# refresh-bio/KMC

Measured on NVIDIA H100. Metric: stage-2 k-mers/s (k=31), higher is better.
Workload: dtype u64

## Files before the change

kmc_b200/csrc/expand.cuh:

```cuda
#pragma once
#include "common.cuh"

#ifndef KMCB200_EXPAND_UNROLL
#define KMCB200_EXPAND_UNROLL 8
#endif

namespace kmcb {

constexpr int kExpandUnroll = KMCB200_EXPAND_UNROLL;

#ifndef KMCB200_EXPAND_IPT
#define KMCB200_EXPAND_IPT 8
#endif
template <int WORDS> struct ExpandCfg { static constexpr int kTile = WORDS == 1 ? 4096 : 2048, kThreads = WORDS == 1 ? 4096 / KMCB200_EXPAND_IPT : 256; };
constexpr int kExpandMinTile = 2048;

struct ExpandArgs {
	const uint8_t* bin;
	uint64_t size;
	const uint64_t* pack_start;
	uint32_t n_packs;
	uint32_t k;
	uint32_t min_rec_bytes;
	uint32_t tile;
	uint32_t both_strands;
	uint64_t n_rec;
	uint32_t* sk_off;
	uint32_t* sk_kpre;
	uint32_t* tile_first;
	uint32_t* pack_nsk;
	uint32_t* pack_nk;
	uint64_t* pack_kbase;
	uint32_t* pack_tbase;
	uint32_t* tile_pack;
	uint4* tile_desc;
	uint64_t tile_pack_cap;
	uint32_t* status;
	uint32_t* flags;
	void* recs;
	uint16_t* cells1;
	uint64_t* item_lo1;
	uint16_t* item_cnt1;
	uint32_t top_shift;
	const uint32_t* cell_scan;
	uint32_t mode;
	uint32_t fshift, fprefix, fmask;
	uint64_t* hist12;
	unsigned long long* out_counter;
	const uint16_t* blk_of_prefix;
	const uint64_t* region_start;
	uint32_t n_blocks;
};
enum : uint32_t { kExpandAll = 0, kExpandCount12 = 1, kExpandFilter = 2, kExpandScatter = 3, kExpandCells = 4, kExpandPartition = 5 };
template <int WORDS> __host__ __device__ constexpr bool expand_partition_supported() { return WORDS == 1; }
constexpr uint32_t kExpandMaxBlocks = 512;
constexpr uint64_t kExpandUnknownRecs = ~0ull;

enum : uint32_t { kErrPackWalk = 1, kErrRecCount = 2 };
constexpr uint32_t kExpandAbortFlag = 2;

__device__ __forceinline__ uint64_t tile_first_base(uint64_t pack_start, uint32_t p, uint32_t tile) { return pack_start * 4 / tile + p; }

constexpr int kWalkSegBytes = 256;
constexpr int kWalkSegs = 256;
constexpr int kWalkChunk = kWalkSegBytes * kWalkSegs;
#ifndef KMCB200_WALK_SPEC
#define KMCB200_WALK_SPEC 1024
#endif
constexpr int kWalkSpec = KMCB200_WALK_SPEC;

__global__ void __launch_bounds__(kWalkSegs, 3) walk_packs_parallel_kernel(const ExpandArgs a, uint32_t* pack_done)
{
	extern __shared__ __align__(16) uint8_t wsm[];
	__shared__ uint32_t s_entry[kWalkSegs], s_exit[kWalkSegs], s_w[16];
	__shared__ uint32_t s_bad;
	const uint32_t p = blockIdx.x, tid = threadIdx.x, lane = tid & 31, warp = tid >> 5;
	const uint64_t pstart = a.pack_start[p];
	const uint32_t len = (uint32_t)min(a.pack_start[p + 1] - pstart, (uint64_t)kWalkChunk + 1);
	if (len > (uint32_t)kWalkChunk || len == 0) { if (tid == 0) pack_done[p] = len == 0 ? 1u : 0u; if (len == 0 && tid == 0) { a.pack_nsk[p] = 0; a.pack_nk[p] = 0; } return; }
	{
		const uintptr_t g0 = reinterpret_cast<uintptr_t>(a.bin + pstart);
		const uintptr_t g0a = g0 & ~(uintptr_t)15;
		const uint32_t shift = (uint32_t)(g0 - g0a);
		const uint32_t nvec = (len + shift + 15) >> 4;
		for (uint32_t v0 = tid; v0 < nvec; v0 += 8 * kWalkSegs) {
			uint4 r[8];
#pragma unroll
			for (int i = 0; i < 8; ++i) { const uint32_t v = v0 + i * kWalkSegs; r[i] = v < nvec ? __ldg(reinterpret_cast<const uint4*>(g0a) + v) : make_uint4(0, 0, 0, 0); }
#pragma unroll
			for (int i = 0; i < 8; ++i) { const uint32_t v = v0 + i * kWalkSegs; if (v < nvec) reinterpret_cast<uint4*>(wsm)[v] = r[i]; }
		}
		if (tid == 0) s_bad = 0;
		__syncthreads();
		const uint8_t* pk = wsm + shift;
		const uint32_t k3 = a.k + 3;
		const uint32_t seg_lo = tid * kWalkSegBytes, seg_hi = min(seg_lo + (uint32_t)kWalkSegBytes, len);
		uint32_t pos = seg_lo > (uint32_t)kWalkSpec ? seg_lo - kWalkSpec : 0;
		if (seg_lo < len) {
			while (pos < seg_lo) pos += 1 + ((pk[pos] + k3) >> 2);
		} else pos = len;
		uint32_t entry = min(pos, len);
		uint32_t nrec = 0, nk = 0;
		pos = entry;
		while (pos < seg_hi) { const uint32_t x = pk[pos]; nk += x + 1; ++nrec; pos += 1 + ((x + k3) >> 2); }
		s_entry[tid] = entry; s_exit[tid] = seg_lo < len ? pos : len;
		for (int it = 0; it < kWalkSegs; ++it) {
			__syncthreads();
			const uint32_t want = tid > 0 ? min(s_exit[tid - 1], len) : 0u;
			const bool fix = tid > 0 && seg_lo < len && entry != want;
			if (!__syncthreads_or(fix)) break;
			if (fix) {
				entry = want; nrec = 0; nk = 0; pos = entry;
				while (pos < seg_hi) { const uint32_t x = pk[pos]; nk += x + 1; ++nrec; pos += 1 + ((x + k3) >> 2); }
				s_entry[tid] = entry; s_exit[tid] = pos;
			}
		}
		__syncthreads();
		bool bad = false;
		if (tid > 0 && seg_lo < len && s_entry[tid] != min(s_exit[tid - 1], len)) bad = true;
		if (tid == kWalkSegs - 1 || seg_hi == len) { if (seg_lo < len && s_exit[tid] != len) bad = true; }
		if (bad) atomicOr(&s_bad, 1u);
		uint32_t ir = nrec, ik = nk;
#pragma unroll
		for (int o = 1; o < 32; o <<= 1) {
			const uint32_t tr = __shfl_up_sync(0xffffffffu, ir, o), tk = __shfl_up_sync(0xffffffffu, ik, o);
			if (lane >= (uint32_t)o) { ir += tr; ik += tk; }
		}
		if (lane == 31) { s_w[warp] = ir; s_w[8 + warp] = ik; }
		__syncthreads();
		if (s_bad) {
			if (tid == 0) { atomicOr(a.status, kErrPackWalk); a.pack_nsk[p] = 0; a.pack_nk[p] = 0; pack_done[p] = 1; }
			return;
		}
		uint32_t br = ir - nrec, bk = ik - nk, tr = 0, tk = 0;
#pragma unroll
		for (int w = 0; w < 8; ++w) { if ((uint32_t)w < warp) { br += s_w[w]; bk += s_w[8 + w]; } tr += s_w[w]; tk += s_w[8 + w]; }
		const uint64_t slot = pstart / a.min_rec_bytes;
		const uint64_t tfb = tile_first_base(pstart, p, a.tile);
		uint32_t j = br, kk = bk;
		pos = entry;
		while (pos < seg_hi) {
			const uint32_t x = pk[pos];
			a.sk_off[slot + j] = (uint32_t)(pstart + pos);
			a.sk_kpre[slot + j] = kk;
			const uint32_t tb = (kk + a.tile - 1) / a.tile;
			if (tb * a.tile < kk + x + 1) a.tile_first[tfb + tb] = j;
			kk += x + 1;
			pos += 1 + ((x + k3) >> 2);
			++j;
		}
		if (tid == 0) { a.pack_nsk[p] = tr; a.pack_nk[p] = tk; pack_done[p] = 1; }
	}
}

constexpr int kWalkWarpsPerBlock = 4;

__device__ __forceinline__ uint4 walk_load_window(const uint8_t* bin_aligned, uint64_t wbase, uint64_t limit, uint32_t lane)
{
	const uint64_t o = wbase + 16ull * lane;
	return o < limit ? __ldg(reinterpret_cast<const uint4*>(bin_aligned + o)) : make_uint4(0, 0, 0, 0);
}

__global__ void __launch_bounds__(32 * kWalkWarpsPerBlock) walk_packs_kernel(const ExpandArgs a, const uint32_t* pack_done)
{
	const uint32_t lane = threadIdx.x & 31u;
	const uint32_t p = blockIdx.x * kWalkWarpsPerBlock + (threadIdx.x >> 5);
	if (p >= a.n_packs) return;
	if (pack_done && pack_done[p]) return;
	uint64_t pos = a.pack_start[p];
	const uint64_t end = a.pack_start[p + 1];
	const uint64_t slot = pos / a.min_rec_bytes;
	const uint64_t tfb = tile_first_base(pos, p, a.tile);
	const uintptr_t base_addr = reinterpret_cast<uintptr_t>(a.bin);
	const uint8_t* bin_aligned = reinterpret_cast<const uint8_t*>(base_addr & ~(uintptr_t)15);
	const uint64_t shift = base_addr & 15u;
	const uint64_t limit = ((a.size + shift + 15) & ~15ull);
	uint64_t wbase = (pos + shift) & ~511ull;
	uint4 cur = walk_load_window(bin_aligned, wbase, limit, lane);
	uint4 nxt = walk_load_window(bin_aligned, wbase + 512, limit, lane);
	uint32_t j = 0, nk = 0, next_tile = 0;
	uint32_t my_off = 0, my_kpre = 0;
	while (pos < end) {
		uint64_t rel = pos + shift - wbase;
		if (rel >= 512) {
			cur = nxt;
			wbase += 512;
			nxt = walk_load_window(bin_aligned, wbase + 512, limit, lane);
			rel -= 512;
		}
		const uint32_t r = (uint32_t)rel;
		const uint32_t comp = (r >> 2) & 3u;
		uint32_t w = comp == 0 ? cur.x : comp == 1 ? cur.y : comp == 2 ? cur.z : cur.w;
		w = __shfl_sync(0xffffffffu, w, r >> 4);
		const uint32_t x = (w >> ((r & 3u) * 8u)) & 0xFFu;
		if (lane == (j & 31u)) { my_off = (uint32_t)pos; my_kpre = nk; }
		if ((j & 31u) == 31u) {
			a.sk_off[slot + j - 31 + lane] = my_off;
			a.sk_kpre[slot + j - 31 + lane] = my_kpre;
		}
		if (nk + x + 1 > next_tile * a.tile) {
			if (lane == 0) a.tile_first[tfb + next_tile] = j;
			++next_tile;
		}
		nk += x + 1;
		pos += 1 + ((x + a.k + 3) >> 2);
		++j;
	}
	if (lane < (j & 31u)) {
		a.sk_off[slot + (j & ~31u) + lane] = my_off;
		a.sk_kpre[slot + (j & ~31u) + lane] = my_kpre;
	}
	if (lane == 0) {
		if (pos != end) atomicOr(a.status, kErrPackWalk);
		a.pack_nsk[p] = j;
		a.pack_nk[p] = nk;
	}
}

__global__ void __launch_bounds__(1024) index_from_extras_kernel(const ExpandArgs a, const uint8_t* __restrict__ extras, const uint64_t* __restrict__ pack_rec_start)
{
	__shared__ uint32_t s_b[32], s_k[32];
	__shared__ uint32_t carry_b, carry_k;
	__shared__ uint32_t s_bad;
	const uint32_t p = blockIdx.x, tid = threadIdx.x, lane = tid & 31, warp = tid >> 5;
	const uint64_t pstart = a.pack_start[p];
	const uint32_t len = (uint32_t)min(a.pack_start[p + 1] - pstart, (uint64_t)0xffffffffu);
	const uint64_t r0 = pack_rec_start[p];
	const uint32_t nrec = (uint32_t)min(pack_rec_start[p + 1] - r0, (uint64_t)0xffffffffu);
	const uint64_t slot = pstart / a.min_rec_bytes;
	const uint64_t tfb = tile_first_base(pstart, p, a.tile);
	if (tid == 0) { carry_b = 0; carry_k = 0; s_bad = 0; }
	__syncthreads();
	const bool too_many = (uint64_t)nrec * a.min_rec_bytes > (uint64_t)len;
	for (uint32_t j0 = 0; j0 < nrec && !too_many; j0 += 1024) {
		const uint32_t j = j0 + tid;
		const uint32_t x = j < nrec ? extras[r0 + j] : 0u;
		const uint32_t nb = j < nrec ? 1u + ((x + a.k + 3u) >> 2) : 0u, nk = j < nrec ? x + 1u : 0u;
		uint32_t ib = nb, ik = nk;
#pragma unroll
		for (int o = 1; o < 32; o <<= 1) {
			const uint32_t tb = __shfl_up_sync(0xffffffffu, ib, o), tk = __shfl_up_sync(0xffffffffu, ik, o);
			if (lane >= (uint32_t)o) { ib += tb; ik += tk; }
		}
		if (lane == 31) { s_b[warp] = ib; s_k[warp] = ik; }
		__syncthreads();
		uint32_t bb = carry_b, bk = carry_k;
		for (uint32_t w = 0; w < warp; ++w) { bb += s_b[w]; bk += s_k[w]; }
		const uint32_t off = bb + ib - nb, kk = bk + ik - nk;
		if (j < nrec) {
			if (off + nb > len || a.bin[pstart + off] != (uint8_t)x) atomicOr(&s_bad, 1u);
			else {
				a.sk_off[slot + j] = (uint32_t)(pstart + off);
				a.sk_kpre[slot + j] = kk;
				const uint32_t tb = (kk + a.tile - 1) / a.tile;
				if (tb * a.tile < kk + x + 1) a.tile_first[tfb + tb] = j;
			}
		}
		__syncthreads();
		if (tid == 1023) { carry_b = bb + ib; carry_k = bk + ik; }
		__syncthreads();
	}
	if (tid == 0) {
		const bool bad = too_many || s_bad || carry_b != len;
		if (bad) atomicOr(a.status, kErrPackWalk);
		a.pack_nsk[p] = bad ? 0u : nrec;
		a.pack_nk[p] = bad ? 0u : carry_k;
	}
}

__global__ void __launch_bounds__(1024) scan_packs_kernel(const ExpandArgs a)
{
	__shared__ uint64_t s_k[32];
	__shared__ uint32_t s_t[32];
	__shared__ uint64_t carry_k;
	__shared__ uint32_t carry_t;
	const uint32_t tid = threadIdx.x, lane = tid & 31, warp = tid >> 5;
	if (tid == 0) { carry_k = 0; carry_t = 0; }
	__syncthreads();
	const bool walk_failed = (a.status[0] & kErrPackWalk) != 0;
	for (uint32_t base = 0; base < a.n_packs && !walk_failed; base += 1024) {
		const uint32_t p = base + tid;
		const uint32_t nk = p < a.n_packs ? a.pack_nk[p] : 0;
		const uint32_t nt = (nk + a.tile - 1) / a.tile;
		uint64_t ik = nk;
		uint32_t it = nt;
#pragma unroll
		for (int o = 1; o < 32; o <<= 1) {
			uint64_t tk = __shfl_up_sync(0xffffffffu, ik, o);
			uint32_t tt = __shfl_up_sync(0xffffffffu, it, o);
			if (lane >= (uint32_t)o) { ik += tk; it += tt; }
		}
		if (lane == 31) { s_k[warp] = ik; s_t[warp] = it; }
		__syncthreads();
		uint64_t bk = carry_k;
		uint32_t bt = carry_t;
		for (uint32_t w = 0; w < warp; ++w) { bk += s_k[w]; bt += s_t[w]; }
		const uint64_t ek = bk + ik - nk;
		const uint32_t et = bt + it - nt;
		if (p < a.n_packs) {
			a.pack_kbase[p] = ek;
			a.pack_tbase[p] = et;
			for (uint32_t t = 0; t < nt && (uint64_t)et + t < a.tile_pack_cap; ++t) a.tile_pack[et + t] = p;
		}
		__syncthreads();
		if (tid == 1023) { carry_k = ek + nk; carry_t = et + nt; }
		__syncthreads();
	}
	if (tid == 0) {
		a.pack_kbase[a.n_packs] = carry_k;
		a.pack_tbase[a.n_packs] = carry_t;
		bool bad = walk_failed;
		if (a.n_rec != kExpandUnknownRecs && carry_k != a.n_rec) { atomicOr(a.status, kErrRecCount); bad = true; }
		if ((uint64_t)carry_t > a.tile_pack_cap) bad = true;
		a.status[1] = bad ? 0u : carry_t;
		if (bad && a.flags) { atomicOr(&a.flags[0], kExpandAbortFlag); atomicOr(&a.flags[1], kExpandAbortFlag); }
	}
}

__global__ void __launch_bounds__(256) tile_desc_kernel(const ExpandArgs a)
{
	const uint32_t g = blockIdx.x * 256 + threadIdx.x;
	if (g >= a.status[1]) return;
	const uint32_t p = a.tile_pack[g];
	const uint32_t t = g - a.pack_tbase[p];
	const uint64_t pstart = a.pack_start[p];
	const uint64_t slot0 = pstart / a.min_rec_bytes;
	const uint32_t nk = a.pack_nk[p];
	const uint32_t tile_start = t * a.tile;
	const uint32_t cnt = min(a.tile, nk - tile_start);
	const uint32_t j_lo = a.tile_first[tile_first_base(pstart, p, a.tile) + t];
	const uint64_t obase = a.pack_kbase[p] + tile_start;
	a.tile_desc[2 * (size_t)g] = make_uint4((uint32_t)slot0, a.pack_nsk[p], j_lo, a.sk_off[slot0 + j_lo]);
	a.tile_desc[2 * (size_t)g + 1] = make_uint4(tile_start | (cnt - 1u), (uint32_t)a.pack_start[p + 1], (uint32_t)obase, (uint32_t)(obase >> 32));
}

__device__ __forceinline__ uint64_t bswap64(uint64_t x)
{
	const uint32_t lo = (uint32_t)x, hi = (uint32_t)(x >> 32);
	return ((uint64_t)__byte_perm(lo, 0, 0x0123) << 32) | (uint64_t)__byte_perm(hi, 0, 0x0123);
}
__device__ __forceinline__ uint64_t rev_symbols64(uint64_t x)
{
	const uint64_t y = __brevll(x);
	return ((y >> 1) & 0x5555555555555555ull) | ((y & 0x5555555555555555ull) << 1);
}

template <int WORDS, typename Load8>
__device__ __forceinline__ Rec<WORDS> extract_kmer(const uint8_t* payload, uint32_t s, uint32_t k, bool canonical, Load8 load8)
{
	const uint8_t* A = payload + (s >> 2);
	const uint32_t sh = (s & 3u) * 2u;
	const uintptr_t a0 = reinterpret_cast<uintptr_t>(A) & ~(uintptr_t)7;
	const uint32_t bo = (uint32_t)(reinterpret_cast<uintptr_t>(A) - a0) * 8u + sh;
	const uintptr_t need_end = reinterpret_cast<uintptr_t>(A) + ((sh + 2u * k + 7u) >> 3);
	uint64_t b[WORDS + 1];
#pragma unroll
	for (int i = 0; i <= WORDS; ++i) {
		const uintptr_t wa = a0 + 8u * i;
		b[i] = wa < need_end ? bswap64(load8(wa)) : 0ull;
	}
	uint64_t t[WORDS];
#pragma unroll
	for (int i = 0; i < WORDS; ++i) t[i] = bo ? ((b[i] << bo) | (b[i + 1] >> (64u - bo))) : b[i];
	const uint32_t rs = 64u * WORDS - 2u * k;
	Rec<WORDS> f;
#pragma unroll
	for (int i = 0; i < WORDS; ++i) {
		uint64_t v = t[i] >> rs;
		if (i > 0 && rs) v |= t[i - 1] << (64u - rs);
		f.w[WORDS - 1 - i] = v;
	}
	if (!canonical) return f;
	uint64_t u[WORDS];
#pragma unroll
	for (int i = 0; i < WORDS; ++i) u[i] = ~rev_symbols64(f.w[i]);
	Rec<WORDS> r;
#pragma unroll
	for (int i = 0; i < WORDS; ++i) {
		uint64_t v = u[i] >> rs;
		if (i > 0 && rs) v |= u[i - 1] << (64u - rs);
		r.w[WORDS - 1 - i] = v;
	}
	return rec_less<WORDS>(f, r) ? f : r;
}

template <int WORDS>
__device__ __forceinline__ Rec<WORDS> extract_kmer_be32(const uint32_t* sw, uint32_t B, uint32_t k, bool canonical)
{
	const uint32_t wi = B >> 5, bo = B & 31u;
	uint32_t w[2 * WORDS + 1];
#pragma unroll
	for (int i = 0; i <= 2 * WORDS; ++i) w[i] = sw[wi + i];
	uint64_t t[WORDS];
#pragma unroll
	for (int i = 0; i < WORDS; ++i)
		t[i] = ((uint64_t)__funnelshift_l(w[2 * i + 1], w[2 * i], bo) << 32) | (uint64_t)__funnelshift_l(w[2 * i + 2], w[2 * i + 1], bo);
	const uint32_t rs = 64u * WORDS - 2u * k;
	Rec<WORDS> f;
#pragma unroll
	for (int i = 0; i < WORDS; ++i) {
		uint64_t v = t[i] >> rs;
		if (i > 0 && rs) v |= t[i - 1] << (64u - rs);
		f.w[WORDS - 1 - i] = v;
	}
	if (!canonical) return f;
	uint64_t u[WORDS];
#pragma unroll
	for (int i = 0; i < WORDS; ++i) u[i] = ~rev_symbols64(f.w[i]);
	Rec<WORDS> r;
#pragma unroll
	for (int i = 0; i < WORDS; ++i) {
		uint64_t v = u[i] >> rs;
		if (i > 0 && rs) v |= u[i - 1] << (64u - rs);
		r.w[WORDS - 1 - i] = v;
	}
	return rec_less<WORDS>(f, r) ? f : r;
}

template <int WORDS>
__device__ __forceinline__ uint32_t rec_top_digit(const Rec<WORDS>& r, uint32_t shift)
{
	const uint32_t wi = shift >> 6, off = shift & 63u;
	uint64_t lo = r.w[0], hi = 0;
#pragma unroll
	for (int i = 1; i < WORDS; ++i) {
		if (wi == (uint32_t)i) lo = r.w[i];
		if (wi + 1 == (uint32_t)i) hi = r.w[i];
	}
	uint64_t v = lo >> off;
	if (WORDS > 1 && off) v |= hi << (64u - off);
	return (uint32_t)v & 0xFFu;
}

template <int WORDS>
__device__ __forceinline__ uint32_t msd_free_bits(const Rec<WORDS>& r, uint32_t shift, uint32_t mask)
{
	if (WORDS == 1) return (uint32_t)(r.w[0] >> shift) & mask;
	const uint32_t wi = shift >> 6, off = shift & 63u;
	uint64_t lo = r.w[0], hi = 0;
#pragma unroll
	for (int i = 1; i < WORDS; ++i) {
		if (wi == (uint32_t)i) lo = r.w[i];
		if (wi + 1 == (uint32_t)i) hi = r.w[i];
	}
	uint64_t v = lo >> off;
	if (off) v |= hi << (64u - off);
	return (uint32_t)v & mask;
}

template <int WORDS, uint32_t MODE>
__host__ __device__ constexpr int expand_min_blocks() { return MODE == kExpandPartition ? 3 : WORDS <= 2 ? 2048 / ExpandCfg<WORDS>::kThreads : 6; }

template <int WORDS, uint32_t MODE = kExpandAll>
__global__ void __launch_bounds__(ExpandCfg<WORDS>::kThreads, expand_min_blocks<WORDS, MODE>()) expand_kernel(const ExpandArgs a)
{
	constexpr int kExpandTile = ExpandCfg<WORDS>::kTile, kExpandThreads = ExpandCfg<WORDS>::kThreads;
	constexpr int IPT = kExpandTile / kExpandThreads;
	constexpr int MAXSK = 1024, STAGE = 12288;
	constexpr int HW = kExpandTile / 32;
	constexpr int SBYTES = MODE == kExpandPartition && kExpandTile * 8 * WORDS > STAGE + 32 ? kExpandTile * 8 * WORDS : STAGE + 32;
	static_assert(MODE != kExpandPartition || expand_partition_supported<WORDS>(), "kExpandPartition: one-word records only");
	__shared__ uint32_t hbits[HW];
	__shared__ uint32_t hpre[HW];
	__shared__ uint32_t s_bit[MAXSK];
	__shared__ __align__(16) uint8_t s_bytes[SBYTES];
	__shared__ uint32_t s_jmax;
	__shared__ unsigned long long s_fbase;
	__shared__ uint32_t warp_max[kExpandThreads / 32];
	__shared__ uint32_t htop[256];
	static_assert(HW <= 128 && HW % 32 == 0, "the head bitmap is scanned by one warp, HW / 32 words per lane");
	const uint32_t tid = threadIdx.x, lane = tid & 31, warp = tid >> 5;
	const uint32_t le_mask = 0xffffffffu >> (31u - lane);
	static_assert(kExpandThreads % 32 == 0, "output slot i * threads + tid belongs to lane tid % 32");
	if constexpr (MODE == kExpandPartition)
		if (a.flags[1] & kExpandAbortFlag) return;
	if (tid < 256) htop[tid] = 0;
	const uint32_t total_tiles = a.status[1];
	Rec<WORDS>* __restrict__ out = reinterpret_cast<Rec<WORDS>*>(a.recs);

	for (uint32_t g = blockIdx.x; g < total_tiles; g += gridDim.x) {
		uint32_t digit_base = 0;
		if constexpr (MODE == kExpandPartition)
			if (tid < 256) digit_base = __ldg(a.cell_scan + g + (size_t)tid * total_tiles);
		const uint4 da = __ldg(a.tile_desc + 2 * (size_t)g), db = __ldg(a.tile_desc + 2 * (size_t)g + 1);
		if (g + gridDim.x < total_tiles) asm volatile("prefetch.global.L2 [%0];" ::"l"(a.tile_desc + 2 * (size_t)(g + gridDim.x)));
		const uint64_t slot0 = da.x;
		const uint32_t nsk = da.y;
		const uint32_t j_lo = da.z;
		const uint32_t off_lo = da.w;
		const uint32_t tile_start = db.x & ~(uint32_t)(kExpandTile - 1);
		const uint32_t cnt = (db.x & (uint32_t)(kExpandTile - 1)) + 1u;
		const uint32_t* __restrict__ kpre = a.sk_kpre + slot0;
		const uint32_t* __restrict__ off = a.sk_off + slot0;
		const uintptr_t g0a = reinterpret_cast<uintptr_t>(a.bin + off_lo) & ~(uintptr_t)15;
		const uint32_t base_off = (uint32_t)(reinterpret_cast<uintptr_t>(a.bin + off_lo) - g0a);

		__syncthreads();
		if (tid < (uint32_t)HW) hbits[tid] = 0;
		if (tid == 0) s_jmax = j_lo;
		__syncthreads();
		{
			uint32_t jm = j_lo;
			for (uint32_t j = j_lo + tid; j < nsk; j += kExpandThreads) {
				const uint32_t kp = kpre[j];
				if (j > j_lo && kp >= tile_start + cnt) break;
				const uint32_t rel = j - j_lo;
				if (rel < (uint32_t)MAXSK) s_bit[rel] = 8u * (base_off + (off[j] - off_lo) + 1u) + 2u * tile_start - 2u * kp;
				if (j > j_lo) atomicOr(&hbits[(kp - tile_start) >> 5], 1u << ((kp - tile_start) & 31u));
				jm = j;
			}
			if (jm > j_lo) atomicMax(&s_jmax, jm);
		}
		__syncthreads();
		const uint32_t j_hi = s_jmax;
		const uint64_t b_hi = j_hi + 1 < nsk ? (uint64_t)off[j_hi + 1] : (uint64_t)db.y;
		const uint64_t span = reinterpret_cast<uintptr_t>(a.bin + b_hi) - g0a;
		const bool staged = (j_hi - j_lo) < (uint32_t)MAXSK && span + 16 <= (uint64_t)STAGE;
		if (staged)
			for (uint32_t v = tid; v * 16 < span + 8; v += kExpandThreads) {
				uint4 x = __ldg(reinterpret_cast<const uint4*>(g0a) + v);
				x.x = __byte_perm(x.x, 0, 0x0123); x.y = __byte_perm(x.y, 0, 0x0123); x.z = __byte_perm(x.z, 0, 0x0123); x.w = __byte_perm(x.w, 0, 0x0123);
				reinterpret_cast<uint4*>(s_bytes)[v] = x;
			}
		if (warp == 0) {
			constexpr int WPL = HW / 32;
			uint32_t c[WPL], tot = 0;
#pragma unroll
			for (int i = 0; i < WPL; ++i) { c[i] = __popc(hbits[lane * WPL + i]); tot += c[i]; }
			uint32_t inc = tot;
#pragma unroll
			for (int o = 1; o < 32; o <<= 1) {
				const uint32_t x = __shfl_up_sync(0xffffffffu, inc, o);
				if (lane >= (uint32_t)o) inc += x;
			}
			uint32_t ex = inc - tot;
#pragma unroll
			for (int i = 0; i < WPL; ++i) { hpre[lane * WPL + i] = ex; ex += c[i]; }
		}
		__syncthreads();

		const uint64_t obase = ((uint64_t)db.w << 32) | db.z;
		auto kmer_of = [&](uint32_t slot) -> Rec<WORDS> {
			const uint32_t rel = hpre[slot >> 5] + __popc(hbits[slot >> 5] & le_mask);
			if (staged) return extract_kmer_be32<WORDS>(reinterpret_cast<const uint32_t*>(s_bytes), s_bit[rel] + 2u * slot, a.k, a.both_strands != 0);
			const uint32_t j = j_lo + rel;
			const uint32_t s = tile_start + slot - kpre[j];
			return extract_kmer<WORDS>(a.bin + off[j] + 1, s, a.k, a.both_strands != 0,
				[](uintptr_t wa) { return __ldg(reinterpret_cast<const unsigned long long*>(wa)); });
		};
		auto top_digit_of = [&](uint32_t slot) -> uint32_t {
			if (WORDS > 1 || !staged || a.top_shift + 8u != 2u * a.k) return rec_top_digit<WORDS>(kmer_of(slot), a.top_shift);
			const uint32_t rel = hpre[slot >> 5] + __popc(hbits[slot >> 5] & le_mask);
			const uint32_t B = s_bit[rel] + 2u * slot;
			const uint32_t* sw = reinterpret_cast<const uint32_t*>(s_bytes);
			auto byte_at = [&](uint32_t b) { const uint32_t wi = b >> 5; return __funnelshift_l(sw[wi + 1], sw[wi], b & 31u) >> 24; };
			const uint32_t f = byte_at(B);
			if (!a.both_strands) return f;
			uint32_t r = ~byte_at(B + 2u * a.k - 8u) & 0xFFu;
			r = ((r & 0x03u) << 6) | ((r & 0x0Cu) << 2) | ((r & 0x30u) >> 2) | ((r & 0xC0u) >> 6);
			return min(f, r);
		};
		if constexpr (MODE == kExpandAll || MODE == kExpandCells) {
#pragma unroll kExpandUnroll
			for (int i = 0; i < IPT; ++i) {
				const uint32_t slot = i * kExpandThreads + tid;
				if (slot < cnt) {
					if constexpr (MODE == kExpandAll) {
						const Rec<WORDS> r = kmer_of(slot);
						out[obase + slot] = r;
						atomicAdd(&htop[rec_top_digit<WORDS>(r, a.top_shift)], 1u);
					} else atomicAdd(&htop[top_digit_of(slot)], 1u);
				}
			}
			__syncthreads();
			if (tid < 256) {
				a.cells1[(uint64_t)tid * total_tiles + g] = (uint16_t)htop[tid];
				htop[tid] = 0;
			}
			if (tid == 0) { a.item_lo1[g] = obase; a.item_cnt1[g] = (uint16_t)cnt; }
		} else if constexpr (MODE == kExpandPartition) {
			__shared__ uint32_t s_excl[256], s_goff[256];
			Rec<WORDS> key[IPT];
			uint32_t rank[IPT / 2] = {};
#pragma unroll
			for (int i = 0; i < IPT; ++i) {
				const uint32_t slot = i * kExpandThreads + tid;
				if (slot < cnt) {
					key[i] = kmer_of(slot);
					rank[i / 2] |= atomicAdd(&htop[rec_top_digit<WORDS>(key[i], a.top_shift)], 1u) << (16 * (i & 1));
				}
			}
			__syncthreads();
			uint32_t c = 0, inc = 0;
			if (tid < 256) {
				c = htop[tid];
				htop[tid] = 0;
				inc = c;
#pragma unroll
				for (int o = 1; o < 32; o <<= 1) {
					const uint32_t x = __shfl_up_sync(0xffffffffu, inc, o);
					if (lane >= (uint32_t)o) inc += x;
				}
				if (lane == 31) warp_max[warp] = inc;
			}
			__syncthreads();
			if (tid < 256) {
				uint32_t ex = inc - c;
#pragma unroll
				for (int w = 0; w < 8; ++w) if ((uint32_t)w < warp) ex += warp_max[w];
				s_excl[tid] = ex;
				s_goff[tid] = digit_base - ex;
			}
			__syncthreads();
			Rec<WORDS>* buf = reinterpret_cast<Rec<WORDS>*>(s_bytes);
#pragma unroll
			for (int i = 0; i < IPT; ++i) {
				const uint32_t slot = i * kExpandThreads + tid;
				if (slot < cnt) buf[s_excl[rec_top_digit<WORDS>(key[i], a.top_shift)] + ((rank[i / 2] >> (16 * (i & 1))) & 0xFFFFu)] = key[i];
			}
			__syncthreads();
#pragma unroll
			for (int i = 0; i < IPT; ++i) {
				const uint32_t q = i * kExpandThreads + tid;
				if (q < cnt) {
					const Rec<WORDS> r = buf[q];
					out[s_goff[rec_top_digit<WORDS>(r, a.top_shift)] + q] = r;
				}
			}
		} else if constexpr (MODE == kExpandCount12) {
			for (int i = 0; i < IPT; ++i) {
				const uint32_t slot = i * kExpandThreads + tid;
				if (slot < cnt) {
					const Rec<WORDS> r = kmer_of(slot);
					atomicAdd(reinterpret_cast<unsigned long long*>(a.hist12) + msd_free_bits<WORDS>(r, a.fshift, 0xFFFu), 1ull);
				}
			}
		} else if constexpr (MODE == kExpandScatter) {
			__shared__ uint32_t s_bcnt[kExpandMaxBlocks];
			__shared__ unsigned long long s_bbase[kExpandMaxBlocks];
			for (uint32_t b = tid; b < a.n_blocks; b += kExpandThreads) s_bcnt[b] = 0;
			__syncthreads();
			uint16_t blk[IPT], rnk[IPT];
#pragma unroll
			for (int i = 0; i < IPT; ++i) {
				const uint32_t slot = i * kExpandThreads + tid;
				if (slot < cnt) {
					const Rec<WORDS> r = kmer_of(slot);
					blk[i] = a.blk_of_prefix[msd_free_bits<WORDS>(r, a.fshift, 0xFFFu)];
					if (blk[i] != 0xFFFFu) rnk[i] = (uint16_t)atomicAdd(&s_bcnt[blk[i]], 1u);
				}
			}
			__syncthreads();
			for (uint32_t b = tid; b < a.n_blocks; b += kExpandThreads) {
				const uint32_t c = s_bcnt[b];
				if (c) s_bbase[b] = a.region_start[b] + atomicAdd(a.out_counter + b, (unsigned long long)c);
			}
			__syncthreads();
#pragma unroll
			for (int i = 0; i < IPT; ++i) {
				const uint32_t slot = i * kExpandThreads + tid;
				if (slot < cnt && blk[i] != 0xFFFFu) out[s_bbase[blk[i]] + rnk[i]] = kmer_of(slot);
			}
		} else {
			for (int i = 0; i < IPT; ++i) {
				const uint32_t slot = i * kExpandThreads + tid;
				Rec<WORDS> r;
				bool keep = false;
				if (slot < cnt) { r = kmer_of(slot); keep = msd_free_bits<WORDS>(r, a.fshift, a.fmask) == a.fprefix; }
				const uint32_t bal = __ballot_sync(0xffffffffu, keep);
				__syncthreads();
				if (lane == 0) warp_max[warp] = __popc(bal);
				__syncthreads();
				if (tid == 0) {
					uint32_t tot = 0;
					for (int w = 0; w < kExpandThreads / 32; ++w) { const uint32_t c = warp_max[w]; warp_max[w] = tot; tot += c; }
					s_fbase = tot ? atomicAdd(a.out_counter, (unsigned long long)tot) : 0ull;
				}
				__syncthreads();
				if (keep) out[s_fbase + warp_max[warp] + __popc(bal & lanemask_lt())] = r;
			}
		}
	}
}

}
```

kmc_b200/csrc/kmc_b200.cu:

```cuda
#include "../../include/kmc_b200.h"
#include "common.cuh"
#include "expand.cuh"
#include "radix_sort.cuh"
#include "count.cuh"
#include "msd_sort.cuh"
#include "leaf_warp.cuh"
#include "leaf_hash.cuh"
#include "leaf_hash_cta.cuh"
#include "leaf_hash_wide.cuh"
#include "split.cuh"
#include "fastx.cuh"
#include "small_k.cuh"

#include <cmath>
#include <cstddef>
#include <cstdarg>
#include <cstdio>
#include <cstdlib>
#include <cstring>
#include <string>
#include <vector>
#include <algorithm>
#include <list>
#include <thread>

using namespace kmcb;

namespace {

constexpr int kMaxPasses = 4 * 8;
constexpr int kHistRows = kMaxPasses + 1;
constexpr int kCounterSlots = kMaxPasses + 8;
constexpr uint32_t kEpochLimit = (1u << 22) - 2;
constexpr int kStageRing = 4;
constexpr size_t kMaxLeaves = 256 * 1024;
constexpr uint32_t kHeavyListCap = 2048;

thread_local std::string g_create_error;

enum { kHistNone = 0, kHistTiles = 1, kHistCells = 2 };

struct ZeroBlock {
	uint64_t hist[kHistRows][256];
	uint32_t counters[kCounterSlots];
	uint32_t status[2];
	uint32_t msd_flags[4];
	uint32_t msd_n_items[2];
	uint32_t msd_counters[4];
	uint32_t heavy_count[2];
	uint32_t heavy_list[kHeavyListCap];
	uint32_t leaf_group_sum[kMaxLeaves / 1024];
};

static_assert(sizeof(ZeroBlock) % 4 == 0, "zeroed word by word");

struct Slot {
	cudaStream_t stream = nullptr;
	uint8_t* recs_a = nullptr; size_t recs_a_cap = 0;
	uint8_t* recs_b = nullptr; size_t recs_b_cap = 0;
	uint8_t* recs_x = nullptr; size_t recs_x_cap = 0;
	uint8_t* d_bin = nullptr; size_t bin_cap = 0;
	uint64_t* d_pack_start = nullptr; size_t packs_cap = 0;
	uint64_t* h_pack_start[kStageRing] = {}; cudaEvent_t ev_pack[kStageRing] = {}; int ring = 0;
	uint32_t* pack_nsk = nullptr; uint32_t* pack_nk = nullptr; uint32_t* pack_tbase = nullptr; uint64_t* pack_kbase = nullptr;
	uint32_t* pack_done = nullptr;
	uint32_t* sk_off = nullptr; size_t sk_off_cap = 0;
	uint32_t* sk_kpre = nullptr; size_t sk_kpre_cap = 0;
	uint32_t* tile_first = nullptr; size_t tile_first_cap = 0;
	uint32_t* tile_pack = nullptr; size_t tile_pack_cap = 0;
	uint4* tile_desc = nullptr; size_t tile_desc_cap = 0;
	ZeroBlock* zero = nullptr;
	uint64_t* desc = nullptr; size_t desc_cap = 0;
	uint64_t* msd_seg1 = nullptr;
	uint64_t* msd_start2 = nullptr;
	uint64_t* msd_start3 = nullptr;
	uint32_t* msd_item_base1 = nullptr;
	uint32_t* msd_item_base2 = nullptr;
	uint32_t* msd_item_seg2 = nullptr; size_t msd_item_seg2_cap = 0;
	uint64_t* msd_item_lo1 = nullptr; size_t msd_item_lo1_cap = 0;
	uint16_t* msd_item_cnt1 = nullptr; size_t msd_item_cnt1_cap = 0;
	uint16_t* msd_cells = nullptr; size_t msd_cells_cap = 0;
	uint32_t* msd_cell_scan = nullptr; size_t msd_cell_scan_cap = 0;
	uint32_t* msd_block_sums = nullptr; size_t msd_block_sums_cap = 0;
	uint8_t* leaf_tmp = nullptr; size_t leaf_tmp_cap = 0;
	uint32_t* leaf_emit = nullptr; uint64_t* leaf_off = nullptr;
	const char* pass_names[kMaxPasses + 8] = {};
	uint32_t last_n_packs = 1;
	uint64_t* cdesc = nullptr; size_t cdesc_cap = 0;
	int hist_mode = 0;
	ExpandArgs expand_args{};
	uint8_t* d_out = nullptr; size_t out_cap = 0;
	uint64_t* d_lut = nullptr;
	uint64_t* d_result = nullptr; uint64_t* h_result = nullptr; uint64_t* h_result_dev = nullptr;
	cudaEvent_t ev_begin = nullptr, ev_expand = nullptr, ev_sort = nullptr, ev_count = nullptr, ev_result = nullptr;
	cudaEvent_t ev_h2d = nullptr, ev_done = nullptr, ev_walk = nullptr;
	cudaEvent_t ev_pass[kMaxPasses + 8] = {};
	int n_passes_run = 0;
	bool ran_expand = false, ran_sort = false, ran_count = false;
	uint64_t* d_hist12 = nullptr; unsigned long long* d_out_counter = nullptr; size_t out_counter_cap = 0;
	uint16_t* d_blk_of_prefix = nullptr; uint64_t* d_region_start = nullptr; size_t region_cap = 0; bool last_scatter = false;
	uint64_t* tot_lut = nullptr; uint64_t* tot_res = nullptr; uint32_t last_blocks = 0;
	bool scan_lut = false; uint64_t scan_base = 0;
	uint8_t* d_extras = nullptr; size_t extras_cap = 0; uint64_t* d_pack_rec = nullptr; size_t pack_rec_cap = 0;
	uint64_t* h_pack_rec = nullptr; size_t h_pack_rec_cap = 0; bool have_extras = false;
	bool sync_done = false; uint64_t sync_out_bytes = 0; uint64_t sync_stats[4] = {};
	bool busy = false;
	uint8_t* host_out = nullptr; uint64_t host_out_cap = 0; uint64_t* host_lut = nullptr; uint64_t pending_n_rec = 0;
};

}

struct kmcb200_ctx {
	kmcb200_params prm{};
	int words = 1;
	uint32_t key_bytes = 0, suffix_bytes = 0, counter_bytes = 0;
	uint64_t lut_entries = 0;
	int sm_count = 0;
	int occ_radix = 1, occ_expand = 1, occ_expand_part = 1, occ_msd_part = 1, occ_msd_part_wide = 1, occ_msd_local = 1;
	uint32_t force_b2 = 0;
	bool use_msd = true;
	bool scatter_blocks = true;
	uint64_t key_block_records = 1ull << 28;
	bool overlap_walk = true;
	bool use_leaf = true;
	int occ_leaf_hash = 1;
	int leaf_cta = 2;
	int leaf_cta_slot_bits = 12;
	int occ_leaf_cta = 1;
	uint32_t leaf_max_b2 = 8;
	uint32_t leaf_target = 1024;
	uint32_t leaf_fill_pct = 62;
	uint32_t leaf_ratio0_q8 = 90;
	uint64_t max_block_records = 1ull << 28;
	uint64_t max_chunk_bytes = 1ull << 30;
	int leaf_slot_bits = 10;
	uint32_t epoch = 1;
	uint64_t launches = 0;
	cudaStream_t compute = nullptr;
	std::vector<Slot> slots;
	std::string err;
};

namespace {

int fail(kmcb200_ctx* c, int code, const char* fmt, ...)
{
	char buf[512];
	va_list ap;
	va_start(ap, fmt);
	vsnprintf(buf, sizeof buf, fmt, ap);
	va_end(ap);
	if (c) c->err = buf;
	else g_create_error = buf;
	return code;
}

#define CU(call)                                                                                             \
	do {                                                                                                     \
		cudaError_t e_ = (call);                                                                             \
		if (e_ != cudaSuccess) return fail(ctx, KMCB200_ERR_CUDA, "%s failed: %s (%s:%d)", #call, cudaGetErrorString(e_), __FILE__, __LINE__); \
	} while (0)

__global__ void zero_words_kernel(uint32_t* p, size_t n_words)
{
	for (size_t i = (size_t)blockIdx.x * blockDim.x + threadIdx.x; i < n_words; i += (size_t)gridDim.x * blockDim.x) p[i] = 0u;
}
int zero_async(kmcb200_ctx* ctx, void* ptr, size_t bytes, cudaStream_t st)
{
	if (bytes == 0) return 0;
	if ((reinterpret_cast<uintptr_t>(ptr) & 3u) || (bytes & 3u) || bytes > (size_t(1) << 28)) { CU(cudaMemsetAsync(ptr, 0, bytes, st)); return 0; }
	const size_t n = bytes / 4;
	zero_words_kernel<<<(unsigned)std::min<size_t>((n + 255) / 256, 1184), 256, 0, st>>>(reinterpret_cast<uint32_t*>(ptr), n);
	ctx->launches++;
	CU(cudaGetLastError());
	return 0;
}

__global__ void bin_init_kernel(uint32_t* zero_block, uint32_t zero_words, uint32_t* lut, size_t lut_words, uint32_t* result)
{
	const size_t stride = (size_t)gridDim.x * blockDim.x, i0 = (size_t)blockIdx.x * blockDim.x + threadIdx.x;
	for (size_t i = i0; i < zero_words; i += stride) zero_block[i] = 0u;
	if (lut) for (size_t i = i0; i < lut_words; i += stride) lut[i] = 0u;
	if (result && i0 < 16) result[i0] = 0u;
}

uint32_t byte_log(uint64_t x) { return x < (1u << 8) ? 1 : x < (1u << 16) ? 2 : x < (1u << 24) ? 3 : 4; }

template <typename T>
int ensure(kmcb200_ctx* ctx, T*& p, size_t& cap, size_t need_elems, bool zero = false)
{
	if (need_elems <= cap && p) return 0;
	size_t n = std::max<size_t>(need_elems + need_elems / 8, 1024);
	if (p) CU(cudaFree(p));
	p = nullptr; cap = 0;
	CU(cudaMalloc(reinterpret_cast<void**>(&p), n * sizeof(T) + 256));
	if (zero) { CU(cudaMemset(p, 0, n * sizeof(T) + 256)); CU(cudaDeviceSynchronize()); }
	cap = n;
	return 0;
}

int next_epoch(kmcb200_ctx* ctx, uint32_t* out, uint32_t count = 1)
{
	if (ctx->epoch + count >= kEpochLimit) {
		CU(cudaDeviceSynchronize());
		for (auto& s : ctx->slots) {
			if (s.desc) CU(cudaMemset(s.desc, 0, s.desc_cap * sizeof(uint64_t)));
			if (s.cdesc) CU(cudaMemset(s.cdesc, 0, s.cdesc_cap * sizeof(uint64_t)));
		}
		CU(cudaDeviceSynchronize());
		ctx->epoch = 1;
	}
	*out = ctx->epoch;
	ctx->epoch += count;
	return 0;
}

template <int WORDS>
int setup_kernels(kmcb200_ctx* ctx)
{
	CU(cudaFuncSetAttribute(radix_pass_kernel<WORDS>, cudaFuncAttributeMaxDynamicSharedMemorySize, SortSmem<WORDS>::kBytes));
	CU(cudaFuncSetAttribute(lsd_sort_kernel<WORDS>, cudaFuncAttributeMaxDynamicSharedMemorySize, SortSmem<WORDS>::kBytes));
	CU(cudaOccupancyMaxActiveBlocksPerMultiprocessor(&ctx->occ_radix, lsd_sort_kernel<WORDS>, SortCfg<WORDS>::kThreads, SortSmem<WORDS>::kBytes));
	CU(cudaOccupancyMaxActiveBlocksPerMultiprocessor(&ctx->occ_expand, expand_kernel<WORDS>, ExpandCfg<WORDS>::kThreads, 0));
	if constexpr (expand_partition_supported<WORDS>())
		CU((cudaOccupancyMaxActiveBlocksPerMultiprocessor(&ctx->occ_expand_part, expand_kernel<WORDS, kExpandPartition>, ExpandCfg<WORDS>::kThreads, 0)));
	const size_t cs = count_smem_bytes<WORDS>(ctx->suffix_bytes + ctx->counter_bytes);
	CU(cudaFuncSetAttribute(count_emit_kernel<WORDS>, cudaFuncAttributeMaxDynamicSharedMemorySize, (int)cs));
	CU(cudaFuncSetAttribute(msd_partition_kernel<WORDS>, cudaFuncAttributeMaxDynamicSharedMemorySize, MsdSmem<WORDS>::kBytes));
	CU(cudaOccupancyMaxActiveBlocksPerMultiprocessor(&ctx->occ_msd_part, msd_partition_kernel<WORDS>, MsdCfg<WORDS>::kThreads + 32, MsdSmem<WORDS>::kBytes));
	CU(cudaFuncSetAttribute(msd_partition_kernel<WORDS, 1024>, cudaFuncAttributeMaxDynamicSharedMemorySize, MsdSmem<WORDS, 1024>::kBytes));
	CU(cudaOccupancyMaxActiveBlocksPerMultiprocessor(&ctx->occ_msd_part_wide, msd_partition_kernel<WORDS, 1024>, MsdCfg<WORDS>::kThreads + 32, MsdSmem<WORDS, 1024>::kBytes));
	if (ctx->occ_msd_part_wide < 1) ctx->occ_msd_part_wide = 1;
	const int local_smem = msd_local_cap<WORDS>() * 8 * WORDS + (MsdLocalCfg<WORDS>::kThreads / 32) * 1024;
	CU(cudaFuncSetAttribute(msd_local_sort_kernel<WORDS>, cudaFuncAttributeMaxDynamicSharedMemorySize, local_smem));
	CU(cudaOccupancyMaxActiveBlocksPerMultiprocessor(&ctx->occ_msd_local, msd_local_sort_kernel<WORDS>, MsdLocalCfg<WORDS>::kThreads, local_smem));
	if (ctx->occ_radix < 1) ctx->occ_radix = 1;
	if (ctx->occ_expand < 1) ctx->occ_expand = 1;
	if (ctx->occ_msd_part < 1) ctx->occ_msd_part = 1;
	if (ctx->occ_msd_local < 1) ctx->occ_msd_local = 1;
	return 0;
}

template <int WORDS>
int launch_expand(kmcb200_ctx* ctx, const ExpandArgs& a, cudaStream_t st)
{
	const uint64_t n_bound = a.n_rec == kExpandUnknownRecs ? a.size * 4 : a.n_rec;
	const uint32_t max_tiles = (uint32_t)(n_bound / ExpandCfg<WORDS>::kTile) + a.n_packs + 1;
	const uint32_t grid = std::min<uint32_t>(max_tiles, (uint32_t)(ctx->sm_count * (a.mode == kExpandPartition ? std::max(ctx->occ_expand_part, 1) : ctx->occ_expand)));
	switch (a.mode) {
	case kExpandAll: expand_kernel<WORDS, kExpandAll><<<grid, ExpandCfg<WORDS>::kThreads, 0, st>>>(a); break;
	case kExpandCells:
	case kExpandPartition:
		if constexpr (expand_partition_supported<WORDS>()) {
			if (a.mode == kExpandCells) expand_kernel<WORDS, kExpandCells><<<grid, ExpandCfg<WORDS>::kThreads, 0, st>>>(a);
			else expand_kernel<WORDS, kExpandPartition><<<grid, ExpandCfg<WORDS>::kThreads, 0, st>>>(a);
			break;
		} else return fail(ctx, KMCB200_ERR_INVALID, "no level-1 partition expansion for %d-word records", WORDS);
	case kExpandCount12: expand_kernel<WORDS, kExpandCount12><<<grid, ExpandCfg<WORDS>::kThreads, 0, st>>>(a); break;
	case kExpandScatter: expand_kernel<WORDS, kExpandScatter><<<grid, ExpandCfg<WORDS>::kThreads, 0, st>>>(a); break;
	default: expand_kernel<WORDS, kExpandFilter><<<grid, ExpandCfg<WORDS>::kThreads, 0, st>>>(a); break;
	}
	ctx->launches++;
	CU(cudaGetLastError());
	return 0;
}

__global__ void msd_setup_kernel(uint64_t* seg1, uint32_t* item_base1, uint32_t* n_items1, uint64_t n, uint32_t tile)
{
	seg1[0] = 0; seg1[1] = n;
	const uint32_t nt = (uint32_t)((n + tile - 1) / tile);
	item_base1[0] = 0; item_base1[1] = nt;
	*n_items1 = nt;
}

template <int WORDS>
uint32_t choose_b2(const kmcb200_ctx* ctx, uint64_t n, bool counted_leaves)
{
	auto bits_for = [&](uint64_t target) { uint32_t lg = 0; while ((1ull << lg) < (n + target - 1) / target) ++lg; return lg > 8 ? lg - 8 : 0u; };
	uint32_t b2;
	if (counted_leaves) {
		b2 = std::min(bits_for(1024), 10u);
		if (WORDS == 1 && b2 > 8) b2 = std::max(8u, std::min(bits_for(ctx->leaf_target), ctx->leaf_max_b2));
		if (ctx->force_b2) b2 = ctx->force_b2;
	} else
		b2 = std::min(bits_for(std::max<uint64_t>(msd_local_cap<WORDS>() / 5, 64)), 8u);
	return b2;
}
template <int WORDS> uint32_t choose_nd2(const kmcb200_ctx* ctx, uint64_t n, bool counted_leaves) { return 1u << choose_b2<WORDS>(ctx, n, counted_leaves); }

size_t msd_max_items1(uint64_t n_rec, uint32_t n_packs) { return (size_t)(n_rec / kExpandMinTile) + n_packs + 2; }

template <int WORDS>
int ensure_msd(kmcb200_ctx* ctx, Slot& s, uint64_t n, uint32_t n_packs, uint32_t nd2 = 256)
{
	static_assert(msd_tile<WORDS>() >= ExpandCfg<WORDS>::kTile, "a partition tile must hold an expand tile");
	const size_t items1 = std::max(msd_max_items1(n, n_packs), (size_t)(n / msd_tile<WORDS>()) + 2);
	const size_t items2 = (size_t)(n / msd_tile<WORDS>()) + 260;
	const size_t cells = std::max(256 * items1, (size_t)std::max(nd2, 256u) * items2);
	if (int rc = ensure(ctx, s.msd_item_lo1, s.msd_item_lo1_cap, items1)) return rc;
	if (int rc = ensure(ctx, s.msd_item_cnt1, s.msd_item_cnt1_cap, items1)) return rc;
	if (int rc = ensure(ctx, s.msd_item_seg2, s.msd_item_seg2_cap, std::max(items1, items2))) return rc;
	if (int rc = ensure(ctx, s.msd_cells, s.msd_cells_cap, cells)) return rc;
	if (int rc = ensure(ctx, s.msd_cell_scan, s.msd_cell_scan_cap, cells)) return rc;
	if (int rc = ensure(ctx, s.msd_block_sums, s.msd_block_sums_cap, cells / kCellChunk + 2)) return rc;
	return 0;
}

int launch_cell_scan(kmcb200_ctx* ctx, Slot& s, const uint32_t* n_items, uint32_t nd, size_t max_items, const uint32_t* flags, cudaStream_t st)
{
	const uint32_t nb = (uint32_t)(((size_t)nd * max_items + kCellChunk - 1) / kCellChunk);
	cell_reduce_kernel<<<nb, 256, 0, st>>>(s.msd_cells, n_items, nd, s.msd_block_sums, flags);
	cell_scan_sums_kernel<<<1, 1024, 0, st>>>(s.msd_block_sums, n_items, nd, flags);
	cell_scan_kernel<<<nb, 256, 0, st>>>(s.msd_cells, n_items, nd, s.msd_block_sums, s.msd_cell_scan, flags);
	ctx->launches += 3;
	CU(cudaGetLastError());
	return 0;
}

template <int WORDS>
int launch_lsd_sort(kmcb200_ctx* ctx, Slot& s, void* in, void* out, uint64_t n, uint32_t key_bytes, const uint32_t* run_flag, uint32_t run_need,
	uint64_t* reset_lut, uint64_t* reset_result, cudaStream_t st)
{
	constexpr int TILE = SortSmem<WORDS>::kTile;
	LsdSortArgs a{};
	a.a = in; a.b = out; a.n = n; a.n_tiles = (uint32_t)((n + TILE - 1) / TILE); a.key_bytes = key_bytes;
	a.hist = &s.zero->hist[0][0]; a.desc = s.desc; a.tile_counters = s.zero->counters;
	if (int rc = next_epoch(ctx, &a.epoch0, key_bytes)) return rc;
	a.run_flag = run_flag; a.run_need = run_need;
	a.reset_lut = reset_lut; a.reset_lut_entries = ctx->lut_entries; a.reset_result = reset_result;
	const uint32_t grid = std::max(1u, std::min<uint32_t>(a.n_tiles, (uint32_t)(ctx->sm_count * ctx->occ_radix)));
	void* params[] = {&a};
	CU(cudaLaunchCooperativeKernel(reinterpret_cast<const void*>(lsd_sort_kernel<WORDS>), dim3(grid), dim3(SortCfg<WORDS>::kThreads), params, SortSmem<WORDS>::kBytes, st));
	ctx->launches++;
	return 0;
}

struct LeafPlan {
	bool active = false;
	const void* recs = nullptr;
	const uint64_t* start = nullptr;
	uint32_t n_leaves = 0, low_bits = 0;
};

bool msd_path(const kmcb200_ctx* ctx, uint64_t n, uint32_t key_bits) { return ctx->use_msd && key_bits >= 24 && n >= (1u << 16); }

template <int WORDS>
int launch_sort(kmcb200_ctx* ctx, Slot& s, void* a, void* b, uint64_t n, uint32_t key_bytes, uint32_t key_bits, int hist_mode, uint32_t n_packs, cudaStream_t st, bool* result_in_b, LeafPlan* plan = nullptr)
{
	constexpr int TILE = SortSmem<WORDS>::kTile;
	constexpr int MTILE = msd_tile<WORDS>();
	const uint64_t n_tiles64 = (n + TILE - 1) / TILE;
	if (n_tiles64 > 0x7fffffffull || n >= (1ull << 32)) return fail(ctx, KMCB200_ERR_INVALID, "bin too large: %llu records", (unsigned long long)n);
	const uint32_t n_tiles = (uint32_t)n_tiles64;
	const bool msd = msd_path(ctx, n, key_bits);
	if (hist_mode == kHistCells && !msd) return fail(ctx, KMCB200_ERR_INVALID, "the records of this bin were not expanded");
	const uint32_t top_shift = key_bits - 8;
	if (int rc = ensure(ctx, s.desc, s.desc_cap, (size_t)n_tiles * 256, true)) return rc;
	if (msd) if (int rc = ensure_msd<WORDS>(ctx, s, n, n_packs, choose_nd2<WORDS>(ctx, n, plan != nullptr))) return rc;

	const bool hist_ready = hist_mode == kHistTiles || hist_mode == kHistCells;
	if (hist_mode == kHistNone) if (int rc = zero_async(ctx, s.zero, sizeof(ZeroBlock), st)) return rc;
	int iv = 0;
	CU(cudaEventRecord(s.ev_pass[0], st));
	void* lsd_in = a; void* lsd_out = b;
	const uint32_t* lsd_flag = nullptr;
	if (msd) {
		const uint32_t b2 = choose_b2<WORDS>(ctx, n, plan != nullptr);
		const uint32_t nd2 = 1u << b2;
		const uint32_t cap = plan ? (WORDS == 1 ? kLwMaxHeavyLeaf : kLwMaxLeaf) : (uint32_t)msd_local_cap<WORDS>();
		const bool final_in_b = (key_bytes % 2) == 0;
		void* fin = final_in_b ? b : a;
		uint32_t* flags = s.zero->msd_flags;
		const uint32_t* never = &flags[1];
		const size_t max_items1 = hist_ready ? msd_max_items1(n, n_packs) : (size_t)(n / MTILE) + 2;
		const size_t max_items2 = (size_t)(n / MTILE) + 260;
		const uint32_t pgrid1 = (uint32_t)std::min<size_t>(max_items1, (size_t)ctx->sm_count * ctx->occ_msd_part);
		const uint32_t pgrid2 = (uint32_t)std::min<size_t>(max_items2, (size_t)ctx->sm_count * (nd2 > 256 ? ctx->occ_msd_part_wide : ctx->occ_msd_part));
		const int local_smem = msd_local_cap<WORDS>() * 8 * WORDS + (MsdLocalCfg<WORDS>::kThreads / 32) * 1024;

		MsdItems items1{};
		if (hist_ready) {
			items1.item_lo = s.msd_item_lo1; items1.item_cnt = s.msd_item_cnt1; items1.n_items = &s.zero->status[1];
		} else {
			msd_setup_kernel<<<1, 1, 0, st>>>(s.msd_seg1, s.msd_item_base1, &s.zero->msd_n_items[0], n, MTILE);
			items1.seg_start = s.msd_seg1; items1.item_base = s.msd_item_base1; items1.item_seg = s.msd_item_seg2 ;
			items1.n_items = &s.zero->msd_n_items[0];
			if (int rc = zero_async(ctx, s.msd_item_seg2, max_items1 * sizeof(uint32_t), st)) return rc;
			MsdCountArgs c1{a, items1, top_shift, 256, s.msd_cells, never};
			msd_count_kernel<WORDS><<<(uint32_t)std::min<size_t>(max_items1, (size_t)ctx->sm_count * 4), 512, 0, st>>>(c1);
			ctx->launches += 2;
		}
		if (int rc = launch_cell_scan(ctx, s, items1.n_items, 256, max_items1, never, st)) return rc;
		s.pass_names[iv] = "msd_scan_L1"; CU(cudaEventRecord(s.ev_pass[++iv], st));
		MsdBoundsArgs b1{};
		b1.cell_scan = s.msd_cell_scan; b1.items = items1; b1.S = 1; b1.nd = 256; b1.n = n; b1.start = s.msd_start2;
		b1.cap = b2 == 0 ? cap : 0; b1.flags = flags;
		b1.tile = b2 > 0 ? MTILE : 0; b1.item_base = s.msd_item_base2; b1.item_seg = s.msd_item_seg2; b1.n_items = &s.zero->msd_n_items[1];
		MsdPartArgs p1{};
		p1.in = a; p1.out = b; p1.items = items1; p1.cell_scan = s.msd_cell_scan; p1.shift = top_shift; p1.nd = 256;
		p1.flags = never;
		if (hist_mode == kHistCells) {
			ExpandArgs ea = s.expand_args;
			ea.mode = kExpandPartition; ea.recs = b; ea.cell_scan = s.msd_cell_scan;
			if (int rc = launch_expand<WORDS>(ctx, ea, st)) return rc;
			s.pass_names[iv] = "expand_scatter_L1";
		} else {
			msd_partition_kernel<WORDS><<<pgrid1, MsdCfg<WORDS>::kThreads + 32, MsdSmem<WORDS>::kBytes, st>>>(p1);
			ctx->launches++;
			s.pass_names[iv] = "msd_partition_L1";
		}
		CU(cudaEventRecord(s.ev_pass[++iv], st));
		msd_bounds_kernel<<<1, 1024, 0, st>>>(b1);
		ctx->launches++;
		if (b2 > 0) {
			MsdItems items2{};
			items2.seg_start = s.msd_start2; items2.item_base = s.msd_item_base2; items2.item_seg = s.msd_item_seg2; items2.n_items = &s.zero->msd_n_items[1];
			MsdCountArgs c2{b, items2, top_shift - b2, nd2, s.msd_cells, flags};
			if (nd2 > 512) msd_count_kernel<WORDS, 1024><<<(uint32_t)std::min<size_t>(max_items2, (size_t)ctx->sm_count * 4), 512, 0, st>>>(c2);
			else if (nd2 > 256) msd_count_kernel<WORDS, 512><<<(uint32_t)std::min<size_t>(max_items2, (size_t)ctx->sm_count * 4), 512, 0, st>>>(c2);
			else msd_count_kernel<WORDS><<<(uint32_t)std::min<size_t>(max_items2, (size_t)ctx->sm_count * 4), 512, 0, st>>>(c2);
			ctx->launches++;
			if (int rc = launch_cell_scan(ctx, s, items2.n_items, nd2, max_items2, flags, st)) return rc;
			MsdBoundsArgs bb{};
			bb.cell_scan = s.msd_cell_scan; bb.items = items2; bb.S = 256; bb.nd = nd2; bb.n = n; bb.start = s.msd_start3; bb.cap = cap; bb.flags = flags; bb.tile = 0;
			msd_bounds_flat_kernel<<<(256 * nd2 + 256) / 256 + 1, 256, 0, st>>>(bb);
			ctx->launches++;
			s.pass_names[iv] = "msd_count_L2"; CU(cudaEventRecord(s.ev_pass[++iv], st));
			MsdPartArgs p2{};
			p2.in = b; p2.out = a; p2.items = items2; p2.cell_scan = s.msd_cell_scan; p2.shift = top_shift - b2; p2.nd = nd2;
			p2.flags = flags;
			if (nd2 > 256) msd_partition_kernel<WORDS, 1024><<<pgrid2, MsdCfg<WORDS>::kThreads + 32, MsdSmem<WORDS, 1024>::kBytes, st>>>(p2);
			else msd_partition_kernel<WORDS><<<pgrid2, MsdCfg<WORDS>::kThreads + 32, MsdSmem<WORDS>::kBytes, st>>>(p2);
			ctx->launches++;
			s.pass_names[iv] = "msd_partition_L2"; CU(cudaEventRecord(s.ev_pass[++iv], st));
		}
		if (plan) {
			plan->active = true;
			plan->recs = b2 > 0 ? a : b; plan->start = b2 > 0 ? s.msd_start3 : s.msd_start2; plan->n_leaves = 256 * nd2; plan->low_bits = top_shift - b2;
		} else {
			MsdLocalArgs lo{};
			lo.in = b2 > 0 ? a : b; lo.out = fin; lo.start = b2 > 0 ? s.msd_start3 : s.msd_start2; lo.n_buckets = 256 * nd2;
			lo.low_bits = top_shift - b2; lo.bucket_counter = &s.zero->msd_counters[2]; lo.flags = flags;
			const uint32_t lgrid = (uint32_t)std::min<size_t>(lo.n_buckets, (size_t)ctx->sm_count * ctx->occ_msd_local);
			msd_local_sort_kernel<WORDS><<<lgrid, MsdLocalCfg<WORDS>::kThreads, local_smem, st>>>(lo);
			ctx->launches++;
			s.pass_names[iv] = "msd_local_sort"; CU(cudaEventRecord(s.ev_pass[++iv], st));
		}
		lsd_in = b; lsd_out = a; lsd_flag = flags;
		*result_in_b = final_in_b;
	} else
		*result_in_b = (key_bytes % 2) == 1;

	if (plan && plan->active) {
		CU(cudaGetLastError());
		s.n_passes_run = iv;
		return 0;
	}
	if (int rc = launch_lsd_sort<WORDS>(ctx, s, lsd_in, lsd_out, n, key_bytes, msd ? lsd_flag : &s.zero->msd_flags[1], msd ? kMsdFlagFallback : 0u, nullptr, nullptr, st)) return rc;
	s.pass_names[iv] = msd ? "lsd_fallback(all passes)" : "lsd_sort(all passes)"; CU(cudaEventRecord(s.ev_pass[++iv], st));
	CU(cudaGetLastError());
	s.n_passes_run = iv;
	return 0;
}

template <int WORDS>
int launch_count(kmcb200_ctx* ctx, Slot& s, const void* sorted, uint64_t n, uint8_t* d_out, uint64_t out_capacity,
	uint64_t* d_lut, uint64_t* d_result, const uint32_t* run_flag, uint32_t run_need, cudaStream_t st, const uint64_t* out_base = nullptr)
{
	constexpr int TILE = count_tile<WORDS>();
	const uint32_t n_tiles = (uint32_t)((n + TILE - 1) / TILE);
	if (int rc = ensure(ctx, s.cdesc, s.cdesc_cap, (size_t)n_tiles, true)) return rc;
	CountArgs a;
	a.recs = sorted; a.n = n; a.n_tiles = n_tiles; a.k = ctx->prm.kmer_len; a.lut_prefix_len = ctx->prm.lut_prefix_len;
	a.cutoff_min = ctx->prm.cutoff_min; a.cutoff_max = ctx->prm.cutoff_max; a.counter_max = ctx->prm.counter_max;
	a.counter_bytes = ctx->counter_bytes; a.suffix_bytes = ctx->suffix_bytes;
	a.out = d_out; a.out_capacity = out_capacity; a.lut = d_lut; a.result = d_result;
	a.desc = s.cdesc; a.tile_counter = &s.zero->counters[kMaxPasses];
	if (int rc = next_epoch(ctx, &a.epoch)) return rc;
	a.run_flag = run_flag; a.run_need = run_need; a.out_base = out_base;
	const size_t smem = count_smem_bytes<WORDS>(ctx->suffix_bytes + ctx->counter_bytes);
	count_emit_kernel<WORDS><<<std::min<uint32_t>(n_tiles, (uint32_t)ctx->sm_count * 6), CountCfg<WORDS>::kThreads, smem, st>>>(a);
	ctx->launches++;
	CU(cudaGetLastError());
	return 0;
}

#define DISPATCH_WORDS(ctx, fn, ...)                                   \
	((ctx)->words == 1 ? fn<1>(__VA_ARGS__) : (ctx)->words == 2 ? fn<2>(__VA_ARGS__) \
	 : (ctx)->words == 3 ? fn<3>(__VA_ARGS__) : fn<4>(__VA_ARGS__))

int set_device(kmcb200_ctx* ctx) { CU(cudaSetDevice(ctx->prm.device)); return 0; }

int check_slot(kmcb200_ctx* ctx, uint32_t slot)
{
	if (!ctx) return KMCB200_ERR_INVALID;
	if (slot >= ctx->slots.size()) return fail(ctx, KMCB200_ERR_INVALID, "slot %u out of range (n_slots=%zu)", slot, ctx->slots.size());
	return 0;
}

struct ExpandMode {
	uint32_t mode = kExpandAll, fshift = 0, fprefix = 0, fmask = 0xFFFu;
	uint64_t* hist12 = nullptr;
	unsigned long long* out_counter = nullptr;
	const uint16_t* blk_of_prefix = nullptr; const uint64_t* region_start = nullptr; uint32_t n_blocks = 0;
};

int upload_packs(kmcb200_ctx* ctx, Slot& s, uint64_t size, const uint64_t* pack_bytes, uint32_t n_packs, cudaStream_t st)
{
	const uint32_t np = (n_packs && pack_bytes) ? n_packs : 1;
	if (np + 1 > s.packs_cap) {
		const size_t cap = np + np / 4 + 64;
		CU(cudaDeviceSynchronize());
		for (int i = 0; i < kStageRing; ++i) {
			if (s.h_pack_start[i]) CU(cudaFreeHost(s.h_pack_start[i]));
			s.h_pack_start[i] = nullptr;
		}
		for (void* p : {(void*)s.d_pack_start, (void*)s.pack_nsk, (void*)s.pack_nk, (void*)s.pack_tbase, (void*)s.pack_kbase})
			if (p) CU(cudaFree(p));
		s.packs_cap = 0;
		for (int i = 0; i < kStageRing; ++i) CU(cudaHostAlloc(reinterpret_cast<void**>(&s.h_pack_start[i]), cap * 8, cudaHostAllocDefault));
		CU(cudaMalloc(reinterpret_cast<void**>(&s.d_pack_start), cap * 8));
		CU(cudaMalloc(reinterpret_cast<void**>(&s.pack_nsk), cap * 4));
		CU(cudaMalloc(reinterpret_cast<void**>(&s.pack_nk), cap * 4));
		CU(cudaMalloc(reinterpret_cast<void**>(&s.pack_tbase), cap * 4));
		CU(cudaMalloc(reinterpret_cast<void**>(&s.pack_kbase), cap * 8));
		if (s.pack_done) CU(cudaFree(s.pack_done));
		CU(cudaMalloc(reinterpret_cast<void**>(&s.pack_done), cap * 4));
		s.packs_cap = cap;
	}
	s.ring = (s.ring + 1) % kStageRing;
	CU(cudaEventSynchronize(s.ev_pack[s.ring]));
	uint64_t* hps = s.h_pack_start[s.ring];
	uint64_t acc = 0;
	if (n_packs && pack_bytes) {
		for (uint32_t i = 0; i < np; ++i) { hps[i] = acc; acc += pack_bytes[i]; }
	}
	else acc = size;
	hps[0] = 0;
	hps[np] = acc;
	if (acc != size) return fail(ctx, KMCB200_ERR_BIN_FORMAT, "expander packs cover %llu bytes but the bin has %llu", (unsigned long long)acc, (unsigned long long)size);
	CU(cudaMemcpyAsync(s.d_pack_start, hps, (np + 1) * 8, cudaMemcpyHostToDevice, st));
	CU(cudaEventRecord(s.ev_pack[s.ring], st));
	return 0;
}

int stage_expand(kmcb200_ctx* ctx, Slot& s, const uint8_t* d_bin, uint64_t size, uint64_t n_rec,
	const uint64_t* pack_bytes, uint32_t n_packs, void* d_recs, cudaStream_t st, const ExpandMode& em = ExpandMode(), bool packs_uploaded = false,
	uint64_t* zero_lut = nullptr, uint64_t* zero_result = nullptr, cudaStream_t st_walk = nullptr)
{
	cudaStream_t st_expand = st;
	if (st_walk) st = st_walk;
	if (size >= (1ull << 32)) return fail(ctx, KMCB200_ERR_INVALID, "bin of %llu bytes: bins of 4 GiB or more are not supported", (unsigned long long)size);
	const uint32_t k = ctx->prm.kmer_len;
	const uint32_t min_rec = 1 + (k + 3) / 4;
	const uint32_t np = (n_packs && pack_bytes) ? n_packs : 1;
	if (!packs_uploaded) if (int rc = upload_packs(ctx, s, size, pack_bytes, n_packs, st)) return rc;

	bool big_pack = !(n_packs && pack_bytes) && size > (uint64_t)kWalkChunk;
	if (n_packs && pack_bytes) for (uint32_t i = 0; i < n_packs && !big_pack; ++i) big_pack = pack_bytes[i] > (uint64_t)kWalkChunk;
	s.last_n_packs = np;
	const bool cells = em.mode == kExpandAll || em.mode == kExpandCells;
	s.hist_mode = em.mode == kExpandAll ? kHistTiles : em.mode == kExpandCells ? kHistCells : kHistNone;

	if (int rc = ensure(ctx, s.sk_off, s.sk_off_cap, size / min_rec + 2)) return rc;
	if (int rc = ensure(ctx, s.sk_kpre, s.sk_kpre_cap, size / min_rec + 2)) return rc;
	if (int rc = ensure(ctx, s.tile_first, s.tile_first_cap, size * 4 / kExpandMinTile + np + 2)) return rc;
	const uint64_t n_bound = n_rec == kExpandUnknownRecs ? size * 4 : n_rec;
	if (int rc = ensure(ctx, s.tile_pack, s.tile_pack_cap, n_bound / kExpandMinTile + np + 2)) return rc;
	if (int rc = ensure(ctx, s.tile_desc, s.tile_desc_cap, 2 * (n_bound / kExpandMinTile + np + 2))) return rc;

	ExpandArgs a;
	a.bin = d_bin; a.size = size; a.pack_start = s.d_pack_start; a.n_packs = np; a.k = k; a.min_rec_bytes = min_rec;
	a.both_strands = ctx->prm.both_strands; a.n_rec = n_rec;
	a.tile = ctx->words == 1 ? ExpandCfg<1>::kTile : ExpandCfg<2>::kTile;
	a.sk_off = s.sk_off; a.sk_kpre = s.sk_kpre; a.tile_first = s.tile_first; a.pack_nsk = s.pack_nsk; a.pack_nk = s.pack_nk;
	a.pack_kbase = s.pack_kbase; a.pack_tbase = s.pack_tbase; a.tile_pack = s.tile_pack; a.tile_pack_cap = n_bound / kExpandMinTile + np + 2;
	a.tile_desc = s.tile_desc;
	a.status = s.zero->status; a.flags = s.zero->msd_flags;
	a.recs = d_recs;
	a.mode = em.mode; a.fshift = em.fshift; a.fprefix = em.fprefix; a.fmask = em.fmask; a.hist12 = em.hist12; a.out_counter = em.out_counter;
	a.blk_of_prefix = em.blk_of_prefix; a.region_start = em.region_start; a.n_blocks = em.n_blocks;
	if (cells) {
		if (int rc = DISPATCH_WORDS(ctx, ensure_msd, ctx, s, n_rec, np, DISPATCH_WORDS(ctx, choose_nd2, ctx, n_rec, ctx->use_leaf))) return rc;
		a.cells1 = s.msd_cells; a.item_lo1 = s.msd_item_lo1; a.item_cnt1 = s.msd_item_cnt1;
	} else { a.cells1 = nullptr; a.item_lo1 = nullptr; a.item_cnt1 = nullptr; }
	a.top_shift = std::max(2u * k, 8u) - 8u;
	a.cell_scan = nullptr;
	if (em.mode == kExpandCells) s.expand_args = a;

	bin_init_kernel<<<64, 256, 0, st>>>(reinterpret_cast<uint32_t*>(s.zero), (uint32_t)(sizeof(ZeroBlock) / 4), reinterpret_cast<uint32_t*>(zero_lut),
		(size_t)ctx->lut_entries * 2, reinterpret_cast<uint32_t*>(zero_result));
	if (s.have_extras && cells) {
		index_from_extras_kernel<<<np, 1024, 0, st>>>(a, s.d_extras, s.d_pack_rec);
		ctx->launches += 2;
		big_pack = false;
	} else {
		walk_packs_parallel_kernel<<<np, kWalkSegs, kWalkChunk + 32, st>>>(a, s.pack_done);
		ctx->launches += 2;
	}
	if (big_pack) {
		walk_packs_kernel<<<(np + kWalkWarpsPerBlock - 1) / kWalkWarpsPerBlock, 32 * kWalkWarpsPerBlock, 0, st>>>(a, s.pack_done);
		ctx->launches++;
	}
	scan_packs_kernel<<<1, 1024, 0, st>>>(a);
	tile_desc_kernel<<<(uint32_t)((a.tile_pack_cap + 255) / 256), 256, 0, st>>>(a);
	ctx->launches += 2;
	CU(cudaGetLastError());
	if (st_expand != st) {
		CU(cudaEventRecord(s.ev_walk, st));
		CU(cudaStreamWaitEvent(st_expand, s.ev_walk, 0));
	}
	return DISPATCH_WORDS(ctx, launch_expand, ctx, a, st_expand);
}

int stage_count(kmcb200_ctx* ctx, Slot& s, const void* sorted, uint64_t n, uint8_t* d_out, uint64_t out_capacity,
	uint64_t* d_lut, uint64_t* d_result, cudaStream_t st, bool outputs_zeroed = false, bool guarded = false, const uint64_t* out_base = nullptr)
{
	if (!outputs_zeroed) {
		bin_init_kernel<<<64, 256, 0, st>>>(&s.zero->counters[kMaxPasses], 1u, reinterpret_cast<uint32_t*>(d_lut), (size_t)ctx->lut_entries * 2, reinterpret_cast<uint32_t*>(d_result));
		ctx->launches++;
		CU(cudaGetLastError());
	}
	if (n == 0) return 0;
	return DISPATCH_WORDS(ctx, launch_count, ctx, s, sorted, n, d_out, out_capacity, d_lut, d_result, guarded ? &s.zero->msd_flags[1] : nullptr, 0u, st, out_base);
}

__global__ void finish_result_kernel(uint64_t* result, uint64_t n_rec, const uint32_t* status, const uint32_t* msd_flags, volatile uint64_t* host_result)
{
	if (threadIdx.x == 0) {
		result[3] = n_rec;
		result[6] = status ? status[0] : 0;
		result[7] = msd_flags ? (msd_flags[0] & 1u) : 0;
	}
	__syncwarp();
	if (host_result) {
		if (threadIdx.x < 8) host_result[threadIdx.x] = result[threadIdx.x];
		__threadfence_system();
	}
}

template <int NWARPS, int SLOT_BITS>
int launch_leaf_cta(kmcb200_ctx* ctx, const LeafArgs& la, bool simple, cudaStream_t st)
{
	const size_t smem = sizeof(LcSmem<NWARPS, SLOT_BITS>);
	const uint32_t grid = std::min<uint32_t>(la.n_leaves, (uint32_t)(ctx->sm_count * ctx->occ_leaf_cta));
	if (simple) leaf_hash_cta_kernel<NWARPS, SLOT_BITS, true><<<grid, 32 * NWARPS, smem, st>>>(la);
	else leaf_hash_cta_kernel<NWARPS, SLOT_BITS, false><<<grid, 32 * NWARPS, smem, st>>>(la);
	return 0;
}

template <int NWARPS, int SLOT_BITS>
int setup_leaf_cta(kmcb200_ctx* ctx)
{
	const int smem = (int)sizeof(LcSmem<NWARPS, SLOT_BITS>);
	int occ_t = 1, occ_f = 1;
	CU((cudaFuncSetAttribute(leaf_hash_cta_kernel<NWARPS, SLOT_BITS, true>, cudaFuncAttributeMaxDynamicSharedMemorySize, smem)));
	CU((cudaFuncSetAttribute(leaf_hash_cta_kernel<NWARPS, SLOT_BITS, true>, cudaFuncAttributePreferredSharedMemoryCarveout, 100)));
	CU((cudaFuncSetAttribute(leaf_hash_cta_kernel<NWARPS, SLOT_BITS, false>, cudaFuncAttributeMaxDynamicSharedMemorySize, smem)));
	CU((cudaFuncSetAttribute(leaf_hash_cta_kernel<NWARPS, SLOT_BITS, false>, cudaFuncAttributePreferredSharedMemoryCarveout, 100)));
	CU((cudaOccupancyMaxActiveBlocksPerMultiprocessor(&occ_t, leaf_hash_cta_kernel<NWARPS, SLOT_BITS, true>, 32 * NWARPS, smem)));
	CU((cudaOccupancyMaxActiveBlocksPerMultiprocessor(&occ_f, leaf_hash_cta_kernel<NWARPS, SLOT_BITS, false>, 32 * NWARPS, smem)));
	ctx->occ_leaf_cta = std::max(1, std::min(occ_t, occ_f));
	return 0;
}

constexpr uint64_t kLeafCtaMinMean = 1280;

#define DISPATCH_CTA(ctx, fn, ...) ((ctx)->leaf_cta_slot_bits == 10 ? fn<4, 10>(__VA_ARGS__) : fn<4, 12>(__VA_ARGS__))

template <int WORDS, int SLOT_BITS>
int launch_leaves(kmcb200_ctx* ctx, const LeafArgs& la, uint64_t n_rec, cudaStream_t st)
{
	const size_t hsmem = sizeof(LhSmem<SLOT_BITS>) * kLwWarps;
	const uint32_t hgrid = std::min<uint32_t>((la.n_leaves + kLwWarps - 1) / kLwWarps, (uint32_t)(ctx->sm_count * ctx->occ_leaf_hash));
	const uint32_t max_count = WORDS == 1 ? kLwHeavy : kLwMaxLeaf;
	const bool simple = la.cutoff_min >= 2u && la.cutoff_max >= la.cutoff_min && (la.cutoff_max + 1u == 0u || la.cutoff_max + 1u > max_count + 1u);
	if constexpr (WORDS == 1) {
		if (ctx->leaf_cta == 1 || (ctx->leaf_cta == 2 && n_rec > kLeafCtaMinMean * la.n_leaves)) DISPATCH_CTA(ctx, launch_leaf_cta, ctx, la, simple, st);
		else if (simple) leaf_hash_kernel<SLOT_BITS, true><<<hgrid, 32 * kLwWarps, hsmem, st>>>(la);
		else leaf_hash_kernel<SLOT_BITS, false><<<hgrid, 32 * kLwWarps, hsmem, st>>>(la);
	} else {
		if (simple) leaf_hash_wide_kernel<WORDS, SLOT_BITS, true><<<hgrid, 32 * kLwWarps, hsmem, st>>>(la);
		else leaf_hash_wide_kernel<WORDS, SLOT_BITS, false><<<hgrid, 32 * kLwWarps, hsmem, st>>>(la);
	}
	ctx->launches++;
	CU(cudaGetLastError());
	return 0;
}

template <int WORDS, int SLOT_BITS>
int launch_heavy_leaves(kmcb200_ctx* ctx, const LeafArgs& la, cudaStream_t st)
{
	static_assert(WORDS == 1, "only one-word leaves are noted for the heavy launch");
	const size_t smem = sizeof(LwSmem<SLOT_BITS>) * kLwWarps;
	leaf_warp_kernel<SLOT_BITS><<<(uint32_t)ctx->sm_count, 32 * kLwWarps, smem, st>>>(la);
	ctx->launches++;
	CU(cudaGetLastError());
	return 0;
}

template <int WORDS, int SLOT_BITS>
int setup_leaves(kmcb200_ctx* ctx)
{
	const int hsmem = (int)(sizeof(LhSmem<SLOT_BITS>) * kLwWarps);
	int occ_t = 1, occ_f = 1;
	if constexpr (WORDS == 1) {
		CU((cudaFuncSetAttribute(leaf_warp_kernel<SLOT_BITS>, cudaFuncAttributeMaxDynamicSharedMemorySize, (int)(sizeof(LwSmem<SLOT_BITS>) * kLwWarps))));
		CU((cudaFuncSetAttribute(leaf_hash_kernel<SLOT_BITS, true>, cudaFuncAttributeMaxDynamicSharedMemorySize, hsmem)));
		CU((cudaFuncSetAttribute(leaf_hash_kernel<SLOT_BITS, true>, cudaFuncAttributePreferredSharedMemoryCarveout, 100)));
		CU((cudaFuncSetAttribute(leaf_hash_kernel<SLOT_BITS, false>, cudaFuncAttributeMaxDynamicSharedMemorySize, hsmem)));
		CU((cudaFuncSetAttribute(leaf_hash_kernel<SLOT_BITS, false>, cudaFuncAttributePreferredSharedMemoryCarveout, 100)));
		CU((cudaOccupancyMaxActiveBlocksPerMultiprocessor(&occ_t, leaf_hash_kernel<SLOT_BITS, true>, 32 * kLwWarps, hsmem)));
		CU((cudaOccupancyMaxActiveBlocksPerMultiprocessor(&occ_f, leaf_hash_kernel<SLOT_BITS, false>, 32 * kLwWarps, hsmem)));
		if (ctx->leaf_cta)
			if (int rc = DISPATCH_CTA(ctx, setup_leaf_cta, ctx)) return rc;
	} else {
		CU((cudaFuncSetAttribute(leaf_hash_wide_kernel<WORDS, SLOT_BITS, true>, cudaFuncAttributeMaxDynamicSharedMemorySize, hsmem)));
		CU((cudaFuncSetAttribute(leaf_hash_wide_kernel<WORDS, SLOT_BITS, true>, cudaFuncAttributePreferredSharedMemoryCarveout, 100)));
		CU((cudaFuncSetAttribute(leaf_hash_wide_kernel<WORDS, SLOT_BITS, false>, cudaFuncAttributeMaxDynamicSharedMemorySize, hsmem)));
		CU((cudaFuncSetAttribute(leaf_hash_wide_kernel<WORDS, SLOT_BITS, false>, cudaFuncAttributePreferredSharedMemoryCarveout, 100)));
		CU((cudaOccupancyMaxActiveBlocksPerMultiprocessor(&occ_t, leaf_hash_wide_kernel<WORDS, SLOT_BITS, true>, 32 * kLwWarps, hsmem)));
		CU((cudaOccupancyMaxActiveBlocksPerMultiprocessor(&occ_f, leaf_hash_wide_kernel<WORDS, SLOT_BITS, false>, 32 * kLwWarps, hsmem)));
	}
	ctx->occ_leaf_hash = std::max(1, std::min(occ_t, occ_f));
	return 0;
}

#define DISPATCH_SLOTS(ctx, fn, W, ...) ((ctx)->leaf_slot_bits == 8 ? fn<W, 8>(__VA_ARGS__) : (ctx)->leaf_slot_bits == 10 ? fn<W, 10>(__VA_ARGS__) : fn<W, 9>(__VA_ARGS__))

template <int WORDS> int setup_leaves_w(kmcb200_ctx* ctx) { return DISPATCH_SLOTS(ctx, setup_leaves, WORDS, ctx); }

template <int WORDS>
int run_sort_count_leaves(kmcb200_ctx* ctx, Slot& s, uint64_t n_rec, uint32_t np_eff, uint8_t* d_out, uint64_t out_capacity, uint64_t* d_lut, uint64_t* d_result, cudaStream_t st,
	bool from_blocks = false, uint32_t block_bits = 0, uint32_t block_prefix = 0, bool outputs_zeroed = false, const uint64_t* out_base = nullptr,
	void* ra = nullptr, void* rb = nullptr)
{
	if (!ra) ra = s.recs_a;
	if (!rb) rb = s.recs_b;
	bool in_b = false;
	LeafPlan plan;
	if (int rc = launch_sort<WORDS>(ctx, s, ra, rb, n_rec, ctx->key_bytes, 2u * ctx->prm.kmer_len - block_bits, from_blocks ? (int)kHistNone : s.hist_mode, np_eff, st, &in_b, &plan)) return rc;
	if (!plan.active) {
		CU(cudaEventRecord(s.ev_sort, st));
		s.ran_sort = true;
		const void* sorted = in_b ? rb : ra;
		return stage_count(ctx, s, sorted, n_rec, d_out, out_capacity, d_lut, d_result, st, outputs_zeroed, true, out_base);
	}
	const uint32_t ob = ctx->suffix_bytes + ctx->counter_bytes;
	const size_t pad = (size_t)((ob + 7) / 8) * 8;
	if (int rc = ensure(ctx, s.leaf_tmp, s.leaf_tmp_cap, (size_t)n_rec * pad + 64)) return rc;
	if (!outputs_zeroed) {
		bin_init_kernel<<<64, 256, 0, st>>>(nullptr, 0u, reinterpret_cast<uint32_t*>(d_lut), (size_t)ctx->lut_entries * 2, reinterpret_cast<uint32_t*>(d_result));
		ctx->launches++;
	}
	uint32_t* flags = s.zero->msd_flags;
	LeafArgs la{};
	la.recs = plan.recs; la.start = plan.start; la.n_leaves = plan.n_leaves; la.low_bits = plan.low_bits;
	la.fill_pct = ctx->leaf_fill_pct; la.ratio0_q8 = ctx->leaf_ratio0_q8;
	la.leaf_prefix = block_bits ? block_prefix * plan.n_leaves : 0u;
	la.k = ctx->prm.kmer_len; la.lut_prefix_len = ctx->prm.lut_prefix_len; la.cutoff_min = ctx->prm.cutoff_min; la.cutoff_max = ctx->prm.cutoff_max;
	la.counter_max = ctx->prm.counter_max; la.counter_bytes = ctx->counter_bytes; la.suffix_bytes = ctx->suffix_bytes;
	la.heavy_list = s.zero->heavy_list; la.heavy_count = &s.zero->heavy_count[0]; la.heavy_ticket = &s.zero->heavy_count[1]; la.heavy_cap = kHeavyListCap;
	la.tmp = s.leaf_tmp; la.leaf_emit = s.leaf_emit; la.group_sum = s.zero->leaf_group_sum; la.lut = d_lut; la.result = d_result; la.ticket = &s.zero->msd_counters[3]; la.flags = flags;
	if (int rc = DISPATCH_SLOTS(ctx, launch_leaves, WORDS, ctx, la, n_rec, st)) return rc;
	if constexpr (WORDS == 1) {
		if (int rc = DISPATCH_SLOTS(ctx, launch_heavy_leaves, WORDS, ctx, la, st)) return rc;
	}
	leaf_scan_kernel<<<(plan.n_leaves + 1023) / 1024, 1024, 0, st>>>(s.leaf_emit, s.zero->leaf_group_sum, plan.n_leaves, s.leaf_off, d_result, out_capacity, ob, flags, out_base);
	leaf_gather_kernel<<<(plan.n_leaves + 7) / 8, 256, 0, st>>>(s.leaf_tmp, plan.start, s.leaf_emit, s.leaf_off, plan.n_leaves, ob, d_out, d_result, flags, out_base);
	ctx->launches += 2;
	int iv = s.n_passes_run;
	s.pass_names[iv] = "leaf_count"; CU(cudaEventRecord(s.ev_pass[++iv], st));
	if (int rc = launch_lsd_sort<WORDS>(ctx, s, rb, ra, n_rec, ctx->key_bytes, flags, kMsdFlagFallback, d_lut, d_result, st)) return rc;
	s.pass_names[iv] = "lsd_fallback(all passes)"; CU(cudaEventRecord(s.ev_pass[++iv], st));
	s.n_passes_run = iv;
	CU(cudaEventRecord(s.ev_sort, st));
	s.ran_sort = true;
	const void* sorted = (ctx->key_bytes % 2 == 0) ? rb : ra;
	return launch_count<WORDS>(ctx, s, sorted, n_rec, d_out, out_capacity, d_lut, d_result, flags, kMsdFlagFallback, st, out_base);
}

int run_bin(kmcb200_ctx* ctx, Slot& s, const uint8_t* d_bin, uint64_t size, uint64_t n_rec, const uint64_t* pack_bytes, uint32_t n_packs,
	uint8_t* d_out, uint64_t out_capacity, uint64_t* d_lut, uint64_t* d_result, cudaStream_t st, bool packs_uploaded = false, uint64_t* host_result = nullptr,
	cudaStream_t st_walk = nullptr)
{
	const size_t rec_bytes = (size_t)ctx->words * 8;
	s.ran_expand = s.ran_sort = s.ran_count = false;
	CU(cudaEventRecord(s.ev_begin, st));
	if (n_rec == 0 || size == 0) {
		if (n_rec != 0 || size != 0) return fail(ctx, KMCB200_ERR_BIN_FORMAT, "bin with size=%llu but n_rec=%llu", (unsigned long long)size, (unsigned long long)n_rec);
		if (int rc = stage_count(ctx, s, nullptr, 0, d_out, out_capacity, d_lut, d_result, st)) return rc;
		if (host_result) { finish_result_kernel<<<1, 32, 0, st>>>(d_result, 0, nullptr, nullptr, host_result); ctx->launches++; }
		CU(cudaEventRecord(s.ev_expand, st)); CU(cudaEventRecord(s.ev_sort, st)); CU(cudaEventRecord(s.ev_count, st));
		s.n_passes_run = 0;
		return 0;
	}
	if (int rc = ensure(ctx, s.recs_a, s.recs_a_cap, n_rec * rec_bytes)) return rc;
	if (int rc = ensure(ctx, s.recs_b, s.recs_b_cap, n_rec * rec_bytes)) return rc;
	ExpandMode em;
	if (expand_partition_supported<1>() && ctx->words == 1 && n_rec < (1ull << 32) && msd_path(ctx, n_rec, 2u * ctx->prm.kmer_len)) em.mode = kExpandCells;
	if (int rc = stage_expand(ctx, s, d_bin, size, n_rec, pack_bytes, n_packs, s.recs_a, st, em, packs_uploaded, d_lut, d_result, st_walk)) return rc;
	CU(cudaEventRecord(s.ev_expand, st));
	s.ran_expand = true;
	bool in_b = false;
	const uint32_t np_eff = (n_packs && pack_bytes) ? n_packs : 1u;
	if (ctx->use_leaf) {
		if (int rc = DISPATCH_WORDS(ctx, run_sort_count_leaves, ctx, s, n_rec, np_eff, d_out, out_capacity, d_lut, d_result, st, false, 0u, 0u, true)) return rc;
	} else {
		if (int rc = DISPATCH_WORDS(ctx, launch_sort, ctx, s, s.recs_a, s.recs_b, n_rec, ctx->key_bytes, 2u * ctx->prm.kmer_len, s.hist_mode, np_eff, st, &in_b)) return rc;
		CU(cudaEventRecord(s.ev_sort, st));
		s.ran_sort = true;
		const void* sorted = in_b ? s.recs_b : s.recs_a;
		if (int rc = stage_count(ctx, s, sorted, n_rec, d_out, out_capacity, d_lut, d_result, st, true, true)) return rc;
	}
	finish_result_kernel<<<1, 32, 0, st>>>(d_result, n_rec, s.zero->status, s.zero->msd_flags, host_result);
	ctx->launches++;
	CU(cudaEventRecord(s.ev_count, st));
	s.ran_count = true;
	return 0;
}

struct BinChunk { uint32_t pack0, npacks; uint64_t byte0, bytes, dev_off; };
struct KeyBlock { uint32_t prefix, bits; uint64_t n; };

__global__ void accumulate_block_kernel(uint64_t* tot_lut, const uint64_t* blk_lut, uint64_t lut_entries, uint64_t* tot_res, const uint64_t* blk_res,
	const unsigned long long* appended, uint64_t expected)
{
	for (uint64_t i = (uint64_t)blockIdx.x * blockDim.x + threadIdx.x; i < lut_entries; i += (uint64_t)gridDim.x * blockDim.x) tot_lut[i] += blk_lut[i];
	if (blockIdx.x == 0 && threadIdx.x == 0) {
		tot_res[0] += blk_res[0]; tot_res[1] += blk_res[1]; tot_res[2] += blk_res[2];
		tot_res[5] |= blk_res[5]; tot_res[7] |= blk_res[7];
		if (appended && *appended != expected) tot_res[6] |= kErrRecCount;
		tot_res[4] += blk_res[4];
	}
}

int plan_chunks(kmcb200_ctx* ctx, uint64_t size, const uint64_t* pack_bytes, uint32_t n_packs, std::vector<BinChunk>& chunks, uint64_t* dev_bytes)
{
	if (!pack_bytes || n_packs == 0) return fail(ctx, KMCB200_ERR_INVALID, "an oversized bin (%llu bytes) needs its expander packs", (unsigned long long)size);
	BinChunk c{0, 0, 0, 0, 0};
	uint64_t pos = 0, dev = 0;
	for (uint32_t i = 0; i < n_packs; ++i) {
		if (pack_bytes[i] >= ctx->max_chunk_bytes) return fail(ctx, KMCB200_ERR_BIN_FORMAT, "expander pack %u has %llu bytes", i, (unsigned long long)pack_bytes[i]);
		if (c.npacks && c.bytes + pack_bytes[i] > ctx->max_chunk_bytes) { c.dev_off = dev; dev += (c.bytes + 64 + 15) & ~15ull; chunks.push_back(c); c = BinChunk{i, 0, pos, 0, 0}; }
		c.npacks++; c.bytes += pack_bytes[i]; pos += pack_bytes[i];
	}
	if (c.npacks) { c.dev_off = dev; dev += (c.bytes + 64 + 15) & ~15ull; chunks.push_back(c); }
	if (pos != size) return fail(ctx, KMCB200_ERR_BIN_FORMAT, "expander packs cover %llu bytes but the bin has %llu", (unsigned long long)pos, (unsigned long long)size);
	*dev_bytes = dev;
	return 0;
}

int count_top12(kmcb200_ctx* ctx, Slot& s, const std::vector<BinChunk>& chunks, const uint64_t* pack_bytes, std::vector<uint64_t>& hist, cudaStream_t st)
{
	const uint32_t k = ctx->prm.kmer_len;
	if (!s.d_hist12) { CU(cudaMalloc(reinterpret_cast<void**>(&s.d_hist12), 4096 * 8)); }
	if (int rc = zero_async(ctx, s.d_hist12, 4096 * 8, st)) return rc;
	ExpandMode em;
	em.mode = kExpandCount12; em.fshift = 2 * k - 12; em.hist12 = s.d_hist12;
	for (const BinChunk& c : chunks) {
		if (int rc = stage_expand(ctx, s, s.d_bin + c.dev_off, c.bytes, kExpandUnknownRecs, pack_bytes + c.pack0, c.npacks, nullptr, st, em)) return rc;
		uint32_t status = 0;
		CU(cudaMemcpyAsync(&status, s.zero->status, 4, cudaMemcpyDeviceToHost, st));
		CU(cudaStreamSynchronize(st));
		if (status & kErrPackWalk) return fail(ctx, KMCB200_ERR_BIN_FORMAT, "bin format error: an expander pack does not end on a record boundary");
	}
	hist.assign(4096, 0);
	CU(cudaMemcpyAsync(hist.data(), s.d_hist12, 4096 * 8, cudaMemcpyDeviceToHost, st));
	CU(cudaStreamSynchronize(st));
	return 0;
}

int bisect_blocks(kmcb200_ctx* ctx, const std::vector<uint64_t>& hist, uint32_t lo, uint32_t hi, uint64_t max_records, std::vector<KeyBlock>& blocks)
{
	struct Range { uint32_t lo, len; };
	std::vector<Range> todo;
	std::vector<Range> cover;
	for (uint32_t p = lo; p < hi;) {
		uint32_t len = 1;
		while (len < 4096 && (p % (2 * len)) == 0 && p + 2 * len <= hi) len *= 2;
		cover.push_back(Range{p, len});
		p += len;
	}
	for (size_t q = cover.size(); q-- > 0;) todo.push_back(cover[q]);
	while (!todo.empty()) {
		const Range r = todo.back(); todo.pop_back();
		uint64_t cnt = 0;
		for (uint32_t q = r.lo; q < r.lo + r.len; ++q) cnt += hist[q];
		if (cnt == 0) continue;
		if (cnt <= max_records || r.len == 1) {
			if (cnt >= (1ull << 32)) return fail(ctx, KMCB200_ERR_INVALID, "bin too skewed: %llu k-mers share their first 6 symbols", (unsigned long long)cnt);
			uint32_t lg = 0; while ((1u << lg) < r.len) ++lg;
			blocks.push_back(KeyBlock{r.lo >> lg, 12 - lg, cnt});
		} else { todo.push_back(Range{r.lo + r.len / 2, r.len / 2}); todo.push_back(Range{r.lo, r.len / 2}); }
	}
	return 0;
}

int sort_count_block(kmcb200_ctx* ctx, Slot& s, void* region, void* rb, const KeyBlock& b, uint8_t* d_out, uint64_t out_capacity,
	uint64_t* tot_lut, uint64_t* tot_res, const unsigned long long* appended, cudaStream_t st)
{
	const uint32_t k = ctx->prm.kmer_len;
	if (ctx->use_leaf) {
		if (int rc = DISPATCH_WORDS(ctx, run_sort_count_leaves, ctx, s, b.n, 1u, d_out, out_capacity, s.d_lut, s.d_result, st, true, b.bits, b.prefix, false, tot_res + 4, region, rb)) return rc;
	} else {
		bool in_b = false;
		if (int rc = DISPATCH_WORDS(ctx, launch_sort, ctx, s, region, rb, b.n, ctx->key_bytes, 2u * k - b.bits, (int)kHistNone, 1u, st, &in_b)) return rc;
		CU(cudaEventRecord(s.ev_sort, st));
		if (int rc = stage_count(ctx, s, in_b ? rb : region, b.n, d_out, out_capacity, s.d_lut, s.d_result, st, false, false, tot_res + 4)) return rc;
	}
	accumulate_block_kernel<<<64, 256, 0, st>>>(tot_lut, s.d_lut, ctx->lut_entries, tot_res, s.d_result, appended, b.n);
	ctx->launches++;
	CU(cudaGetLastError());
	return 0;
}

int setup_scatter(kmcb200_ctx* ctx, Slot& s, const std::vector<KeyBlock>& blocks, const std::vector<uint64_t>& region_start, cudaStream_t st)
{
	if (!s.d_out_counter || s.out_counter_cap < blocks.size() + 1) {
		if (s.d_out_counter) CU(cudaFree(s.d_out_counter));
		s.d_out_counter = nullptr;
		s.out_counter_cap = std::max<size_t>(blocks.size() + 1, 64);
		CU(cudaMalloc(reinterpret_cast<void**>(&s.d_out_counter), s.out_counter_cap * 8));
	}
	std::vector<uint16_t> h_blk(4096, (uint16_t)0xFFFF);
	for (size_t i = 0; i < blocks.size(); ++i) {
		const uint32_t lo = blocks[i].prefix << (12 - blocks[i].bits), len = 1u << (12 - blocks[i].bits);
		for (uint32_t q = lo; q < lo + len; ++q) h_blk[q] = (uint16_t)i;
	}
	if (!s.d_blk_of_prefix) CU(cudaMalloc(reinterpret_cast<void**>(&s.d_blk_of_prefix), 4096 * 2));
	if (!s.d_region_start || s.region_cap < blocks.size()) {
		if (s.d_region_start) CU(cudaFree(s.d_region_start));
		s.d_region_start = nullptr;
		s.region_cap = std::max<size_t>(blocks.size(), 64);
		CU(cudaMalloc(reinterpret_cast<void**>(&s.d_region_start), s.region_cap * 8));
	}
	CU(cudaMemcpyAsync(s.d_blk_of_prefix, h_blk.data(), 4096 * 2, cudaMemcpyHostToDevice, st));
	CU(cudaMemcpyAsync(s.d_region_start, region_start.data(), blocks.size() * 8, cudaMemcpyHostToDevice, st));
	CU(cudaStreamSynchronize(st));
	return zero_async(ctx, s.d_out_counter, blocks.size() * 8, st);
}

int scatter_chunks(kmcb200_ctx* ctx, Slot& s, const std::vector<BinChunk>& chunks, const uint64_t* pack_bytes, uint32_t n_blocks, void* dst, cudaStream_t st)
{
	ExpandMode es;
	es.mode = kExpandScatter; es.fshift = 2 * ctx->prm.kmer_len - 12; es.out_counter = s.d_out_counter;
	es.blk_of_prefix = s.d_blk_of_prefix; es.region_start = s.d_region_start; es.n_blocks = n_blocks;
	for (const BinChunk& c : chunks)
		if (int rc = stage_expand(ctx, s, s.d_bin + c.dev_off, c.bytes, kExpandUnknownRecs, pack_bytes + c.pack0, c.npacks, dst, st, es)) return rc;
	s.ran_expand = false;
	CU(cudaEventRecord(s.ev_expand, st));
	return 0;
}

int run_key_blocks(kmcb200_ctx* ctx, Slot& s, const std::vector<BinChunk>& chunks, const uint64_t* pack_bytes, const std::vector<KeyBlock>& blocks,
	uint8_t* d_out, uint64_t out_capacity, uint64_t* tot_lut, uint64_t* tot_res, cudaStream_t st)
{
	const uint32_t k = ctx->prm.kmer_len;
	const size_t rec_bytes = (size_t)ctx->words * 8;
	uint64_t max_n = 0, sum_n = 0;
	for (const KeyBlock& b : blocks) { max_n = std::max(max_n, b.n); sum_n += b.n; }
	bool scatter = ctx->scatter_blocks && blocks.size() > 1 && blocks.size() <= kExpandMaxBlocks && 2 * k >= 24;
	if (scatter) {
		size_t free_b = 0, total_b = 0;
		CU(cudaMemGetInfo(&free_b, &total_b));
		const uint64_t have = (uint64_t)free_b + s.recs_a_cap + s.recs_b_cap + s.leaf_tmp_cap;
		const uint64_t need = sum_n * rec_bytes + max_n * (rec_bytes + 8 * ((ctx->suffix_bytes + ctx->counter_bytes + 7) / 8) + 4) + (256ull << 20);
		scatter = need <= (uint64_t)(0.9 * (double)have);
	}
	s.last_scatter = scatter;
	if (scatter) {
		if (int rc = ensure(ctx, s.recs_a, s.recs_a_cap, (sum_n + blocks.size() + 2) * rec_bytes)) return rc;
		if (int rc = ensure(ctx, s.recs_b, s.recs_b_cap, max_n * rec_bytes)) return rc;
		std::vector<uint64_t> h_reg(blocks.size());
		uint64_t acc = 0;
		for (size_t i = 0; i < blocks.size(); ++i) {
			acc = (acc + 1) & ~1ull;
			h_reg[i] = acc; acc += blocks[i].n;
		}
		if (int rc = setup_scatter(ctx, s, blocks, h_reg, st)) return rc;
		if (int rc = scatter_chunks(ctx, s, chunks, pack_bytes, (uint32_t)blocks.size(), s.recs_a, st)) return rc;
		for (size_t i = 0; i < blocks.size(); ++i)
			if (int rc = sort_count_block(ctx, s, s.recs_a + h_reg[i] * rec_bytes, s.recs_b, blocks[i], d_out, out_capacity, tot_lut, tot_res, s.d_out_counter + i, st)) return rc;
		return 0;
	}
	if (!s.d_out_counter) { s.out_counter_cap = 64; CU(cudaMalloc(reinterpret_cast<void**>(&s.d_out_counter), s.out_counter_cap * 8)); }
	if (int rc = ensure(ctx, s.recs_a, s.recs_a_cap, max_n * rec_bytes)) return rc;
	if (int rc = ensure(ctx, s.recs_b, s.recs_b_cap, max_n * rec_bytes)) return rc;
	for (const KeyBlock& b : blocks) {
		if (int rc = zero_async(ctx, s.d_out_counter, 8, st)) return rc;
		ExpandMode ef;
		ef.mode = kExpandFilter; ef.fshift = 2 * k - b.bits; ef.fprefix = b.prefix; ef.out_counter = s.d_out_counter;
		ef.fmask = b.bits ? ((1u << b.bits) - 1u) : 0u;
		if (b.bits == 0) { ef.fshift = 0; ef.fprefix = 0; }
		for (const BinChunk& c : chunks)
			if (int rc = stage_expand(ctx, s, s.d_bin + c.dev_off, c.bytes, kExpandUnknownRecs, pack_bytes + c.pack0, c.npacks, s.recs_a, st, ef)) return rc;
		s.ran_expand = false;
		CU(cudaEventRecord(s.ev_expand, st));
		if (ctx->use_leaf) {
			if (int rc = DISPATCH_WORDS(ctx, run_sort_count_leaves, ctx, s, b.n, 1u, d_out, out_capacity, s.d_lut, s.d_result, st, true, b.bits, b.prefix, false, tot_res + 4)) return rc;
		} else {
			bool in_b = false;
			if (int rc = DISPATCH_WORDS(ctx, launch_sort, ctx, s, s.recs_a, s.recs_b, b.n, ctx->key_bytes, 2u * k - b.bits, (int)kHistNone, 1u, st, &in_b)) return rc;
			CU(cudaEventRecord(s.ev_sort, st));
			if (int rc = stage_count(ctx, s, in_b ? s.recs_b : s.recs_a, b.n, d_out, out_capacity, s.d_lut, s.d_result, st, false, false, tot_res + 4)) return rc;
		}
		accumulate_block_kernel<<<64, 256, 0, st>>>(tot_lut, s.d_lut, ctx->lut_entries, tot_res, s.d_result, s.d_out_counter, b.n);
		ctx->launches++;
		CU(cudaGetLastError());
	}
	return 0;
}

int ensure_totals(kmcb200_ctx* ctx, Slot& s, cudaStream_t st)
{
	if (!s.tot_lut) {
		CU(cudaMalloc(reinterpret_cast<void**>(&s.tot_lut), ctx->lut_entries * 8));
		CU(cudaMalloc(reinterpret_cast<void**>(&s.tot_res), 64));
	}
	if (int rc = zero_async(ctx, s.tot_lut, ctx->lut_entries * 8, st)) return rc;
	return zero_async(ctx, s.tot_res, 64, st);
}

int run_oversized_bin(kmcb200_ctx* ctx, Slot& s, const uint8_t* h_bin, uint64_t size, uint64_t n_rec, const uint64_t* pack_bytes, uint32_t n_packs,
	uint8_t* h_out, uint64_t out_capacity, uint64_t* h_lut, uint64_t* out_bytes, uint64_t stats[4])
{
	cudaStream_t st = ctx->compute;
	const uint32_t k = ctx->prm.kmer_len;
	std::vector<BinChunk> chunks;
	uint64_t dev_bytes = 0;
	if (int rc = plan_chunks(ctx, size, pack_bytes, n_packs, chunks, &dev_bytes)) return rc;
	if (int rc = ensure(ctx, s.d_bin, s.bin_cap, dev_bytes + 64)) return rc;
	for (const BinChunk& c : chunks) CU(cudaMemcpyAsync(s.d_bin + c.dev_off, h_bin + c.byte0, c.bytes, cudaMemcpyHostToDevice, st));
	std::vector<KeyBlock> blocks;
	if (n_rec <= ctx->max_block_records) blocks.push_back(KeyBlock{0, 0, n_rec});
	else {
		if (2 * k < 24) return fail(ctx, KMCB200_ERR_INVALID, "a bin of %llu k-mers with k = %u: key blocks need k >= 12", (unsigned long long)n_rec, k);
		std::vector<uint64_t> hist;
		if (int rc = count_top12(ctx, s, chunks, pack_bytes, hist, st)) return rc;
		uint64_t total = 0;
		for (uint64_t v : hist) total += v;
		if (total != n_rec) return fail(ctx, KMCB200_ERR_BIN_FORMAT, "bin format error: the bin holds %llu k-mers, not n_rec = %llu", (unsigned long long)total, (unsigned long long)n_rec);
		size_t free_b = 0, total_b = 0;
		CU(cudaMemGetInfo(&free_b, &total_b));
		const uint64_t rec_b = (uint64_t)ctx->words * 8;
		const bool fits_once = ctx->scatter_blocks && (double)n_rec * rec_b + (double)ctx->key_block_records * (rec_b + 12) * 1.5 < 0.85 * (double)(free_b + s.recs_a_cap + s.recs_b_cap + s.leaf_tmp_cap);
		const uint64_t limit = fits_once ? std::min(ctx->max_block_records, ctx->key_block_records) : ctx->max_block_records;
		if (int rc = bisect_blocks(ctx, hist, 0, 4096, limit, blocks)) return rc;
		if (blocks.size() > kExpandMaxBlocks) { blocks.clear(); if (int rc = bisect_blocks(ctx, hist, 0, 4096, ctx->max_block_records, blocks)) return rc; }
	}
	const uint32_t ob = ctx->suffix_bytes + ctx->counter_bytes;
	if (int rc = ensure(ctx, s.d_out, s.out_cap, out_capacity + 64)) return rc;
	if (int rc = ensure_totals(ctx, s, st)) return rc;
	if (int rc = run_key_blocks(ctx, s, chunks, pack_bytes, blocks, s.d_out, out_capacity, s.tot_lut, s.tot_res, st)) return rc;
	uint64_t r[8];
	CU(cudaMemcpyAsync(r, s.tot_res, 64, cudaMemcpyDeviceToHost, st));
	CU(cudaStreamSynchronize(st));
	if (r[6]) return fail(ctx, KMCB200_ERR_BIN_FORMAT, "bin format error: the bin does not hold n_rec = %llu k-mers / a pack does not end on a record boundary", (unsigned long long)n_rec);
	const uint64_t bytes = r[4] * (uint64_t)ob;
	if (r[5] || bytes > out_capacity) return fail(ctx, KMCB200_ERR_CAPACITY, "out_capacity %llu too small", (unsigned long long)out_capacity);
	if (bytes) CU(cudaMemcpyAsync(h_out, s.d_out, bytes, cudaMemcpyDeviceToHost, st));
	CU(cudaMemcpyAsync(h_lut, s.tot_lut, ctx->lut_entries * 8, cudaMemcpyDeviceToHost, st));
	CU(cudaStreamSynchronize(st));
	s.last_blocks = (uint32_t)blocks.size();
	if (out_bytes) *out_bytes = bytes;
	if (stats) { stats[0] = r[0]; stats[1] = r[1]; stats[2] = r[2]; stats[3] = n_rec; }
	return 0;
}

}

namespace { __global__ void lut_scan_kernel(uint64_t* lut, uint64_t n, uint64_t base); }

extern "C" {

int kmcb200_create(const kmcb200_params* prm, kmcb200_ctx** out_ctx)
{
	kmcb200_ctx* ctx = nullptr;
	if (!prm || !out_ctx) return fail(ctx, KMCB200_ERR_INVALID, "null argument");
	*out_ctx = nullptr;
	if (prm->kmer_len < 1 || prm->kmer_len > KMCB200_MAX_KMER_LEN)
		return fail(ctx, KMCB200_ERR_INVALID, "kmer_len %u outside 1..%d", prm->kmer_len, KMCB200_MAX_KMER_LEN);
	if (prm->lut_prefix_len < 1 || prm->lut_prefix_len >= prm->kmer_len || prm->lut_prefix_len > 15 || (prm->kmer_len - prm->lut_prefix_len) % 4 != 0)
		return fail(ctx, KMCB200_ERR_INVALID, "lut_prefix_len %u illegal for k=%u: need 1 <= p <= 15, p < k, (k-p) %% 4 == 0 (kmc.h:1434-1469)", prm->lut_prefix_len, prm->kmer_len);
	if (prm->n_slots < 1 || prm->n_slots > KMCB200_MAX_SLOTS) return fail(ctx, KMCB200_ERR_INVALID, "n_slots %u outside 1..%d", prm->n_slots, KMCB200_MAX_SLOTS);
	int n_dev = 0;
	if (cudaGetDeviceCount(&n_dev) != cudaSuccess || n_dev == 0)
		return fail(ctx, KMCB200_ERR_NO_DEVICE, "no CUDA device visible: kmc_b200 has no CPU fallback");
	if (prm->device < 0 || prm->device >= n_dev) return fail(ctx, KMCB200_ERR_NO_DEVICE, "device %d not present (%d visible)", prm->device, n_dev);
	cudaDeviceProp dp;
	if (cudaGetDeviceProperties(&dp, prm->device) != cudaSuccess) return fail(ctx, KMCB200_ERR_CUDA, "cudaGetDeviceProperties failed");
	if (dp.major != 9 || dp.minor != 0) return fail(ctx, KMCB200_ERR_NO_DEVICE, "device %d is sm_%d%d; kmc_b200 is built for sm_90a (H100) only", prm->device, dp.major, dp.minor);

	ctx = new kmcb200_ctx();
	ctx->prm = *prm;
	ctx->words = (int)((prm->kmer_len + 31) / 32);
	ctx->key_bytes = (prm->kmer_len + 3) / 4;
	ctx->suffix_bytes = (prm->kmer_len - prm->lut_prefix_len) / 4;
	ctx->counter_bytes = prm->counter_max == 1 ? 0 : std::min(byte_log(prm->cutoff_max), byte_log(prm->counter_max));
	ctx->lut_entries = 1ull << (2 * prm->lut_prefix_len);
	ctx->sm_count = dp.multiProcessorCount;
	if (const char* e = getenv("KMCB200_SORT")) ctx->use_msd = std::string(e) != "lsd";
	if (const char* e = getenv("KMCB200_LEAF")) ctx->use_leaf = std::string(e) != "sort";
// ... 551 lines not shown
```

kmc_b200/csrc/leaf_warp.cuh:

```cuda
#pragma once
#include "common.cuh"
#include "expand.cuh"
#include "msd_sort.cuh"
#include "count.cuh"

namespace kmcb {

constexpr int kLwWarps = 4;
constexpr uint32_t kLwGroupBits = 6;
constexpr int kLwList = 256;
constexpr uint32_t kLwRing = 256;
constexpr int kLwMinBlocks = 7;
constexpr uint32_t kLwMaxLeaf = 65534;
constexpr uint32_t kLwHeavy = 16384;
constexpr uint32_t kLwMaxHeavyLeaf = 1u << 22;
constexpr uint32_t kLwMaxSplit = 12;
constexpr uint64_t kLwEmpty = ~0ull;

struct LeafArgs {
	const void* recs;
	const uint64_t* start;
	uint32_t n_leaves;
	uint32_t low_bits;
	uint32_t heavy_cap;
	uint32_t fill_pct;
	uint32_t ratio0_q8;
	uint32_t leaf_prefix;
	uint32_t k, lut_prefix_len, cutoff_min, cutoff_max, counter_max, counter_bytes, suffix_bytes;
	uint8_t* tmp;
	uint32_t* leaf_emit;
	uint32_t* group_sum;
	uint64_t* lut;
	uint64_t* result;
	uint32_t* ticket;
	uint32_t* flags;
	uint32_t* heavy_list; uint32_t* heavy_count; uint32_t* heavy_ticket;
};

template <int SLOT_BITS>
struct LwSmem {
	static constexpr int kSlots = 1 << SLOT_BITS;
	uint64_t main[kSlots];
	uint64_t ring[kLwRing];
	uint32_t surv[kSlots / 32];
	uint32_t over[kSlots / 32];
	__device__ __forceinline__ uint16_t* list() { return reinterpret_cast<uint16_t*>(ring); }
};
static_assert(kLwRing * 8 >= kLwList * 2, "the u16 list lives in the ring");

template <int WORDS>
__device__ __forceinline__ Rec<WORDS> lw_load(const Rec<WORDS>* p)
{
	Rec<WORDS> r;
	if (WORDS == 2) {
		const ulonglong2 v = __ldg(reinterpret_cast<const ulonglong2*>(p));
		r.w[0] = v.x; r.w[WORDS - 1] = v.y;
	} else if (WORDS == 4) {
		const ulonglong2 v0 = __ldg(reinterpret_cast<const ulonglong2*>(p)), v1 = __ldg(reinterpret_cast<const ulonglong2*>(p) + 1);
		r.w[0] = v0.x; r.w[1 % WORDS] = v0.y; r.w[2 % WORDS] = v1.x; r.w[3 % WORDS] = v1.y;
	} else {
#pragma unroll
		for (int i = 0; i < WORDS; ++i) r.w[i] = __ldg(reinterpret_cast<const unsigned long long*>(p) + i);
	}
	return r;
}

template <int WORDS>
__device__ __forceinline__ uint64_t lw_extract64(const Rec<WORDS>& r, uint32_t pos)
{
	const uint32_t wi = pos >> 6, off = pos & 63u;
	uint64_t lo = r.w[0], hi = 0;
#pragma unroll
	for (int i = 1; i < WORDS; ++i) {
		if (wi == (uint32_t)i) lo = r.w[i];
		if (wi + 1 == (uint32_t)i) hi = r.w[i];
	}
	if (WORDS == 1 || wi + 1 >= (uint32_t)WORDS) hi = 0;
	uint64_t v = lo >> off;
	if (off) v |= hi << (64u - off);
	return v;
}

template <int WORDS>
__device__ __forceinline__ uint64_t lw_out_word(const Rec<WORDS>& key, uint32_t value, uint32_t sb, uint32_t w)
{
	const int nkb = (int)sb - 8 * (int)w;
	if (nkb >= 8) return bswap64(lw_extract64<WORDS>(key, 8u * (uint32_t)(nkb - 8)));
	if (nkb > 0) return bswap64(key.w[0] << (8 * (8 - nkb))) | ((uint64_t)value << (8 * nkb));
	const int sh = -nkb;
	return sh < 4 ? (uint64_t)(value >> (8 * sh)) : 0ull;
}

struct LwCut {
	uint32_t cmin;
	uint32_t cmax1;
	bool never;
};
__device__ __forceinline__ void lw_transition(const LwCut& c, uint32_t newc, uint32_t* reached, uint32_t* over, uint32_t idx, uint32_t& r_max)
{
	if (newc != c.cmin && newc != c.cmax1) return;
	if (newc == c.cmin) {
		if (c.never) ++r_max;
		else atomicOr(&reached[idx >> 5], 1u << (idx & 31u));
	}
	if (newc == c.cmax1 && !c.never) { atomicOr(&over[idx >> 5], 1u << (idx & 31u)); ++r_max; }
}

struct LwRound {
	uint64_t* main; uint32_t* surv; uint32_t* over;
	uint32_t gshift, gmask, cb, cmask;
	uint64_t rem_mask;
	LwCut cut;
};

__device__ __forceinline__ uint32_t lw_slot(uint64_t kmer, uint64_t rem, uint32_t gshift, uint32_t gmask)
{
	return ((((uint32_t)(kmer >> gshift)) & gmask) << kLwGroupBits) | ((((uint32_t)rem ^ (uint32_t)(rem >> 27)) * 0x9E3779B1u) >> (32 - kLwGroupBits));
}

template <int V>
__device__ __forceinline__ void lw_insert1(const LwRound& t, const uint64_t (&kk)[V], uint32_t vmask, uint32_t& r_claim, uint32_t& r_max, bool& ok)
{
	constexpr uint32_t GM = (1u << kLwGroupBits) - 1u;
	uint32_t slot[V];
	unsigned long long old[V], ent[V];
#pragma unroll
	for (int v = 0; v < V; ++v) {
		const uint64_t rem = kk[v] & t.rem_mask;
		slot[v] = lw_slot(kk[v], rem, t.gshift, t.gmask);
		ent[v] = (rem << t.cb) | 1ull;
		old[v] = kLwEmpty;
		if ((vmask >> v) & 1u) old[v] = atomicCAS(reinterpret_cast<unsigned long long*>(&t.main[slot[v]]), (unsigned long long)kLwEmpty, ent[v]);
	}
#pragma unroll
	for (int v = 0; v < V; ++v) {
		const bool act = (vmask >> v) & 1u;
		const unsigned long long tag = ent[v] >> t.cb;
		uint32_t s = slot[v];
		unsigned long long o = old[v];
		uint32_t probe = 0;
		while (o != kLwEmpty && (o >> t.cb) != tag) {
			if (++probe > GM) break;
			s = (s & ~GM) | ((s + 1u) & GM);
			o = atomicCAS(reinterpret_cast<unsigned long long*>(&t.main[s]), (unsigned long long)kLwEmpty, ent[v]);
		}
		if (probe > GM) ok = false;
		else if (act) {
			uint32_t newc = 1u;
			if (o == kLwEmpty) ++r_claim;
			else newc = (atomicAdd(reinterpret_cast<uint32_t*>(&t.main[s]), 1u) & t.cmask) + 1u;
			lw_transition(t.cut, newc, t.surv, t.over, s, r_max);
		}
	}
}

template <int SLOT_BITS>
__global__ void __launch_bounds__(32 * kLwWarps, kLwMinBlocks) leaf_warp_kernel(const LeafArgs a)
{
	using R = Rec<1>;
	using SM = LwSmem<SLOT_BITS>;
	constexpr int SLOTS = SM::kSlots;
	constexpr int NW = SLOTS / 32;
	constexpr int NG = SLOTS >> kLwGroupBits;
	constexpr uint32_t GB = SLOT_BITS - kLwGroupBits;
	constexpr uint32_t GM = (1u << kLwGroupBits) - 1u;
	constexpr uint32_t ROUND = SLOTS;
	constexpr uint32_t FULL = 0xffffffffu;
	static_assert(NW <= 32 && NW >= 4, "one bitmap word per lane");
	extern __shared__ __align__(16) uint8_t lw_dsm[];
	SM& S = reinterpret_cast<SM*>(lw_dsm)[threadIdx.x >> 5];
	if (*a.flags & kMsdFlagStop) return;
	const uint32_t lane = threadIdx.x & 31u, lt = lanemask_lt();
	const R* __restrict__ recs = reinterpret_cast<const R*>(a.recs);
	const uint32_t ob = a.suffix_bytes + a.counter_bytes;
	const uint32_t padw = (ob + 7) >> 3;
	const uint32_t prefix_shift = 2u * (a.k - a.lut_prefix_len);
	const bool one_prefix = prefix_shift >= a.low_bits;
	const LwCut cut{a.cutoff_min > 1u ? a.cutoff_min : 1u, a.cutoff_max + 1u, a.cutoff_max < (a.cutoff_min > 1u ? a.cutoff_min : 1u)};
	uint64_t* const tmp64 = reinterpret_cast<uint64_t*>(a.tmp);
	uint16_t* const list = S.list();
	uint32_t t_unique = 0, t_max = 0, t_emit = 0;
	bool failed = false;

	const uint32_t n_work = min(*a.heavy_count, a.heavy_cap);
	uint32_t work = 0;
	if (lane == 0) work = atomicAdd(a.heavy_ticket, 1u);
	work = __shfl_sync(FULL, work, 0);
	while (work < n_work) {
		uint32_t next_t = 0;
		if (lane == 0) next_t = atomicAdd(a.heavy_ticket, 1u);
		const uint32_t leaf = a.heavy_list[work];
		const uint64_t lo = a.start[leaf];
		const uint32_t m = (uint32_t)min(a.start[leaf + 1] - lo, (uint64_t)0xffffffffu);
		uint32_t emit_base = 0;
		bool heavy = false;
		uint64_t cand = 0;
		uint32_t n_eq = 0, m_rest = m;
		const unsigned long long* __restrict__ g = reinterpret_cast<const unsigned long long*>(recs) + lo;
		if (m > kLwHeavy && m <= kLwMaxHeavyLeaf) {
			cand = __ldg(g);
			for (uint32_t j0 = 0; j0 < m; j0 += 128) {
				uint64_t v[4];
#pragma unroll
				for (int u = 0; u < 4; ++u) { const uint32_t j = j0 + u * 32 + lane; v[u] = j < m ? __ldg(g + j) : ~cand; }
#pragma unroll
				for (int u = 0; u < 4; ++u) n_eq += __popc(__ballot_sync(FULL, v[u] == cand));
			}
			heavy = n_eq > m / 4;
			if (heavy) m_rest = m - n_eq; else n_eq = 0;
		}
		if (m_rest > kLwMaxLeaf) failed = true;
		else if (m > 0) {
			uint32_t e0 = 0;
			while (((m_rest >> e0) > ROUND && e0 < 8 && e0 < a.low_bits) || a.low_bits - e0 > GB + 47u) ++e0;
			uint32_t e = e0, r = 0;
			while (true) {
				const uint32_t sub_shift = a.low_bits - e;
				const uint32_t gshift = sub_shift > GB ? sub_shift - GB : 0;
				const uint32_t cb = min(64u - gshift, 32u);
				const uint64_t rem_mask = (1ull << gshift) - 1ull;
				const uint32_t cmask = cb >= 32 ? 0xffffffffu : ((1u << cb) - 1u);
				const uint32_t emask = (1u << e) - 1u;
				{
					const uint4 ev = make_uint4(~0u, ~0u, ~0u, ~0u), zv = make_uint4(0, 0, 0, 0);
#pragma unroll
					for (int i = 0; i < SLOTS * 8 / 16 / 32; ++i) reinterpret_cast<uint4*>(S.main)[i * 32 + lane] = ev;
					if (lane < 2 * NW / 4) reinterpret_cast<uint4*>(S.surv)[lane] = zv;
				}
				__syncwarp();
				uint32_t r_claim = 0, r_max = 0;
				bool ok = true;
				{
					const LwRound T{S.main, S.surv, S.over, gshift, (uint32_t)NG - 1u, cb, cmask, rem_mask, cut};
					uint32_t head = 0, tail = 0;
					uint64_t nx[4];
#pragma unroll
					for (int u = 0; u < 4; ++u) { const uint32_t j = u * 32 + lane; nx[u] = j < m ? __ldg(g + j) : 0ull; }
					for (uint32_t j0 = 0; j0 < m && ok; j0 += 128) {
						uint64_t cur[4];
						bool in[4];
#pragma unroll
						for (int u = 0; u < 4; ++u) { cur[u] = nx[u]; in[u] = (j0 + u * 32 + lane < m) && ((uint32_t)(cur[u] >> sub_shift) & emask) == r && !(heavy && cur[u] == cand); }
#pragma unroll
						for (int u = 0; u < 4; ++u) { const uint32_t j = j0 + 128 + u * 32 + lane; nx[u] = j < m ? __ldg(g + j) : 0ull; }
#pragma unroll
						for (int u = 0; u < 4; ++u) {
							const uint32_t bal = __ballot_sync(FULL, in[u]);
							if (in[u]) S.ring[(tail + __popc(bal & lt)) & (kLwRing - 1)] = cur[u];
							tail += __popc(bal);
						}
						const bool last = j0 + 128 >= m;
						while (tail - head >= 64 || (last && tail != head)) {
							const uint32_t avail = tail - head;
							__syncwarp();
							const uint64_t kk[2] = {S.ring[(head + lane) & (kLwRing - 1)], S.ring[(head + 32 + lane) & (kLwRing - 1)]};
							__syncwarp();
							head += min(avail, 64u);
							lw_insert1<2>(T, kk, (lane < avail ? 1u : 0u) | (32 + lane < avail ? 2u : 0u), r_claim, r_max, ok);
							ok = __all_sync(FULL, ok);
							if (!ok) break;
						}
					}
				}
				if (heavy && ok && ((uint32_t)(cand >> sub_shift) & emask) == r) {
					if (cb < 32 && (n_eq >> cb)) ok = false;
					else if (lane == 0) {
						const uint64_t rem = cand & rem_mask;
						uint32_t sl = lw_slot(cand, rem, gshift, (uint32_t)NG - 1u);
						const unsigned long long ent = (rem << cb) | (unsigned long long)n_eq;
						uint32_t probe = 0;
						while (atomicCAS(reinterpret_cast<unsigned long long*>(&S.main[sl]), (unsigned long long)kLwEmpty, ent) != kLwEmpty) {
							if (++probe > GM) break;
							sl = (sl & ~GM) | ((sl + 1u) & GM);
						}
						if (probe > GM) ok = false;
						else {
							++r_claim;
							if (n_eq >= cut.cmin) { if (cut.never) ++r_max; else atomicOr(&S.surv[sl >> 5], 1u << (sl & 31u)); }
							if (!cut.never && cut.cmax1 != 0u && n_eq >= cut.cmax1) { atomicOr(&S.over[sl >> 5], 1u << (sl & 31u)); ++r_max; }
						}
					}
				}
				__syncwarp();
				ok = __all_sync(FULL, ok);
				if (!ok) {
					if (e < a.low_bits && e < e0 + kLwMaxSplit) { ++e; r <<= 1; continue; }
					failed = true;
					break;
				}
				t_unique += r_claim;
				t_max += r_max;
				const uint64_t key_hi = (gshift + GB) >= 64 ? 0ull
					: (((((uint64_t)(a.leaf_prefix | leaf) << a.low_bits) | ((uint64_t)r << sub_shift)) >> (gshift + GB)) << (gshift + GB));
				auto entry_key = [&](uint32_t s, uint64_t ent) -> R {
					R kk;
					kk.w[0] = key_hi | ((uint64_t)(s >> kLwGroupBits) << gshift) | ((ent >> cb) & rem_mask);
					return kk;
				};
				const uint32_t w_main = lane < (uint32_t)NW ? (S.surv[lane] & ~S.over[lane]) : 0u;
				uint32_t inc = __popc(w_main);
#pragma unroll
				for (int o = 1; o < 32; o <<= 1) {
					const uint32_t t = __shfl_up_sync(FULL, inc, o);
					if (lane >= (uint32_t)o) inc += t;
				}
				const uint32_t w_excl = inc - __popc(w_main);
				const uint32_t n_main = __shfl_sync(FULL, inc, 31);
				__syncwarp();
				if (lane < (uint32_t)NW) { S.surv[lane] = w_main; S.over[lane] = w_excl; }
				for (uint32_t q0 = 0; q0 < n_main; q0 += kLwList) {
					__syncwarp();
					{
						uint32_t w = w_main, q = w_excl;
						while (w) {
							const uint32_t b = __ffs(w) - 1;
							w &= w - 1;
							if (q - q0 < (uint32_t)kLwList) list[q - q0] = (uint16_t)(lane * 32 + b);
							++q;
						}
					}
					__syncwarp();
					const uint32_t q1 = min(n_main, q0 + (uint32_t)kLwList);
					for (uint32_t q = q0 + lane; q < q1; q += 32) {
						const uint32_t s = list[q - q0];
						const uint64_t ent = S.main[s];
						const R kk = entry_key(s, ent);
						const uint32_t w0 = (s >> kLwGroupBits) << (kLwGroupBits - 5);
						uint32_t pos = S.over[w0];
#pragma unroll
						for (uint32_t wi = 0; wi < (1u << (kLwGroupBits - 5)); ++wi) {
							uint32_t others = S.surv[w0 + wi];
							if (w0 + wi == (s >> 5)) others &= ~(1u << (s & 31u));
							while (others) {
								const uint32_t s2 = ((w0 + wi) << 5) | (uint32_t)(__ffs(others) - 1);
								others &= others - 1;
								pos += rec_less<1>(entry_key(s2, S.main[s2]), kk) ? 1u : 0u;
							}
						}
						const uint32_t c = (uint32_t)ent & cmask;
						const uint32_t value = c > a.counter_max ? a.counter_max : c;
						uint64_t* dst = tmp64 + (lo + emit_base + pos) * padw;
						for (uint32_t w = 0; w < padw; ++w) dst[w] = lw_out_word<1>(kk, value, a.suffix_bytes, w);
						if (!one_prefix) atomicAdd(reinterpret_cast<unsigned long long*>(a.lut) + rec_prefix<1>(kk, prefix_shift), 1ull);
					}
				}
				emit_base += n_main;
				__syncwarp();
				while (e > e0 && (r & 1u)) { r >>= 1; --e; }
				++r;
				if (e == e0 && r == (1u << e0)) break;
			}
		}
		if (lane == 0) {
			a.leaf_emit[leaf] = failed ? 0u : emit_base;
			if (emit_base && !failed) atomicAdd(&a.group_sum[leaf >> 10], emit_base);
			t_emit += emit_base;
			if (one_prefix && emit_base && !failed)
				atomicAdd(reinterpret_cast<unsigned long long*>(a.lut) + ((a.leaf_prefix | leaf) >> (prefix_shift - a.low_bits)), (unsigned long long)emit_base);
		}
		if (failed) break;
		work = __shfl_sync(FULL, next_t, 0);
	}
	failed = __any_sync(FULL, failed);
	if (failed) { if (lane == 0) atomicOr(a.flags, kMsdFlagFallback); return; }
#pragma unroll
	for (int o = 16; o > 0; o >>= 1) {
		t_unique += __shfl_down_sync(FULL, t_unique, o);
		t_max += __shfl_down_sync(FULL, t_max, o);
	}
	if (lane == 0) {
		if (t_unique) atomicAdd(reinterpret_cast<unsigned long long*>(a.result), (unsigned long long)t_unique);
		if (t_unique - t_emit - t_max) atomicAdd(reinterpret_cast<unsigned long long*>(a.result) + 1, (unsigned long long)(t_unique - t_emit - t_max));
		if (t_max) atomicAdd(reinterpret_cast<unsigned long long*>(a.result) + 2, (unsigned long long)t_max);
	}
}

__global__ void __launch_bounds__(1024) leaf_scan_kernel(const uint32_t* leaf_emit, const uint32_t* group_sum, uint32_t n_leaves, uint64_t* leaf_off,
	uint64_t* result, uint64_t out_capacity, uint32_t ob, const uint32_t* flags, const uint64_t* out_base)
{
	__shared__ uint32_t s_w[32];
	__shared__ unsigned long long s_base;
	if (*flags & kMsdFlagStop) return;
	const uint32_t tid = threadIdx.x, lane = tid & 31, warp = tid >> 5, g = blockIdx.x, n_groups = gridDim.x;
	if (warp == 0) {
		unsigned long long b = 0, t = 0;
		for (uint32_t j = lane; j < n_groups; j += 32) { const uint32_t v = group_sum[j]; t += v; if (j < g) b += v; }
#pragma unroll
		for (int o = 16; o > 0; o >>= 1) { b += __shfl_xor_sync(0xffffffffu, b, o); t += __shfl_xor_sync(0xffffffffu, t, o); }
		if (lane == 0) {
			s_base = b;
			if (g == 0) { result[4] = t; if (t * ob > out_capacity) result[5] = 1; }
		}
	}
	const uint32_t i = g * 1024 + tid;
	const uint32_t v = i < n_leaves ? leaf_emit[i] : 0u;
	uint32_t inc = v;
#pragma unroll
	for (int o = 1; o < 32; o <<= 1) {
		const uint32_t t = __shfl_up_sync(0xffffffffu, inc, o);
		if (lane >= (uint32_t)o) inc += t;
	}
	if (lane == 31) s_w[warp] = inc;
	__syncthreads();
	unsigned long long base = s_base;
	for (uint32_t w = 0; w < warp; ++w) base += s_w[w];
	if (i < n_leaves) leaf_off[i] = base + inc - v;
}

__global__ void __launch_bounds__(256) leaf_gather_kernel(const uint8_t* tmp, const uint64_t* start, const uint32_t* leaf_emit, const uint64_t* leaf_off,
	uint32_t n_leaves, uint32_t ob, uint8_t* out, const uint64_t* result, const uint32_t* flags, const uint64_t* out_base)
{
	if (*flags & kMsdFlagStop) return;
	if (result[5]) return;
	const uint32_t leaf = blockIdx.x * 8 + (threadIdx.x >> 5), lane = threadIdx.x & 31u;
	if (leaf >= n_leaves) return;
	const uint32_t pad = ((ob + 7) >> 3) << 3;
	const uint32_t nbytes = leaf_emit[leaf] * ob;
	const uint8_t* src = tmp + start[leaf] * pad;
	uint8_t* dst = out + ((out_base ? *out_base : 0ull) + leaf_off[leaf]) * ob;
	if (ob <= 8) {
		const uint32_t n = leaf_emit[leaf];
		const unsigned long long* src8 = reinterpret_cast<const unsigned long long*>(src);
		for (uint32_t r0 = 0; r0 < n; r0 += 64) {
			unsigned long long v[2];
#pragma unroll
			for (int u = 0; u < 2; ++u) { const uint32_t r = r0 + u * 32 + lane; v[u] = r < n ? __ldg(src8 + r) : 0ull; }
#pragma unroll
			for (int u = 0; u < 2; ++u) {
				const uint32_t r = r0 + u * 32 + lane;
				if (r < n) {
					uint8_t* d = dst + (size_t)r * ob;
					for (uint32_t b = 0; b < ob; ++b) d[b] = (uint8_t)(v[u] >> (8 * b));
				}
			}
		}
		return;
	}
	const uint32_t magic = 0xFFFFFFFFu / ob + 1;
	const bool use_magic = nbytes < 65536u && ob > 1;
	for (uint32_t p0 = lane; p0 < nbytes; p0 += 128) {
		uint8_t v[4];
#pragma unroll
		for (int i = 0; i < 4; ++i) {
			const uint32_t p = p0 + 32 * i;
			const uint32_t r = use_magic ? __umulhi(p, magic) : p / ob;
			v[i] = p < nbytes ? __ldg(src + (size_t)r * pad + (p - r * ob)) : (uint8_t)0;
		}
#pragma unroll
		for (int i = 0; i < 4; ++i) {
			const uint32_t p = p0 + 32 * i;
			if (p < nbytes) dst[p] = v[i];
		}
	}
}

}
```

kmc_b200/csrc/msd_sort.cuh:

```cuda
#pragma once
#include "common.cuh"
#include "radix_sort.cuh"

namespace kmcb {

constexpr uint32_t kMsdFlagFallback = 1;
constexpr uint32_t kMsdFlagAbort = 2;
constexpr uint32_t kMsdFlagStop = kMsdFlagFallback | kMsdFlagAbort;

template <int WORDS>
__device__ __forceinline__ uint32_t rec_bits(const Rec<WORDS>& r, uint32_t shift, uint32_t mask)
{
	if (WORDS == 1) return (uint32_t)(r.w[0] >> shift) & mask;
	const uint32_t wi = shift >> 6, off = shift & 63u;
	uint64_t lo = r.w[0], hi = 0;
#pragma unroll
	for (int i = 1; i < WORDS; ++i) {
		if (wi == (uint32_t)i) lo = r.w[i];
		if (wi + 1 == (uint32_t)i) hi = r.w[i];
	}
	uint64_t v = lo >> off;
	if (off) v |= hi << (64u - off);
	return (uint32_t)v & mask;
}

template <int WORDS> struct MsdCfg;
template <> struct MsdCfg<1> { static constexpr int kThreads = 512, kKpt = 8, kMinBlocks = 2; };
template <> struct MsdCfg<2> { static constexpr int kThreads = 512, kKpt = 4, kMinBlocks = 2; };
template <> struct MsdCfg<3> { static constexpr int kThreads = 512, kKpt = 4, kMinBlocks = 1; };
template <> struct MsdCfg<4> { static constexpr int kThreads = 512, kKpt = 4, kMinBlocks = 1; };
static_assert(true, "");

template <int WORDS> __host__ __device__ constexpr int msd_tile() { return MsdCfg<WORDS>::kThreads * MsdCfg<WORDS>::kKpt; }

struct MsdItems {
	const uint64_t* item_lo;
	const uint16_t* item_cnt;
	const uint64_t* seg_start;
	const uint32_t* item_base;
	const uint32_t* item_seg;
	const uint32_t* n_items;
};

struct MsdItemGeom {
	uint64_t lo, hi;
	uint64_t lo_al;
	uint32_t n_load;
	uint64_t cell0;
	uint32_t cell_stride;
};

template <int WORDS>
__device__ __forceinline__ MsdItemGeom msd_item_geom(const MsdItems& it, uint32_t item, uint32_t nd)
{
	constexpr uint64_t TILE = msd_tile<WORDS>();
	MsdItemGeom g;
	if (it.item_lo) {
		g.lo = it.item_lo[item];
		g.hi = g.lo + it.item_cnt[item];
		g.cell_stride = *it.n_items;
		g.cell0 = item;
	} else {
		const uint32_t seg = it.item_seg[item];
		const uint64_t sb = it.seg_start[seg], se = it.seg_start[seg + 1];
		const uint32_t first_item = it.item_base[seg];
		const uint64_t T = sb / TILE + (item - first_item);
		g.lo = T * TILE > sb ? T * TILE : sb;
		g.hi = (T + 1) * TILE < se ? (T + 1) * TILE : se;
		g.cell_stride = it.item_base[seg + 1] - first_item;
		g.cell0 = (uint64_t)nd * first_item + (item - first_item);
	}
	g.lo_al = g.lo & ~1ull;
	g.n_load = (uint32_t)(((g.hi + 1) & ~1ull) - g.lo_al);
	return g;
}


template <int WORDS, int NDMAX = 256>
struct MsdSmem {
	static constexpr int kThreads = MsdCfg<WORDS>::kThreads;
	static constexpr int kKpt = MsdCfg<WORDS>::kKpt;
	static constexpr int kTile = kThreads * kKpt;
	static constexpr int kRecBytes = 8 * WORDS;
	static constexpr int kStages = NDMAX > 256 ? 2 : 3;
	static constexpr int kBufStride = ((kTile + 2) * kRecBytes + 127) & ~127;
	static constexpr int oBuf = 0;
	static constexpr int oHist = kStages * kBufStride;
	static constexpr int oExcl = oHist + 4 * NDMAX;
	static constexpr int oGoff = oExcl + 4 * NDMAX;
	static constexpr int oBase = oGoff + 4 * NDMAX;
	static constexpr int oWarpTot = oBase + kStages * 4 * NDMAX;
	static constexpr int oGeom = oWarpTot + 64;
	static constexpr int oMbar = oGeom + kStages * 16;
	static constexpr int kBytes = oMbar + 2 * kStages * 8;
};

__device__ __forceinline__ void bar_sync_named(uint32_t id, uint32_t n_threads) { asm volatile("bar.sync %0, %1;" ::"r"(id), "r"(n_threads) : "memory"); }
__device__ __forceinline__ void mbar_arrive(uint64_t* bar) { asm volatile("mbarrier.arrive.shared::cta.b64 _, [%0];" ::"r"(smem_u32(bar)) : "memory"); }

struct MsdPartArgs {
	const void* in;
	void* out;
	MsdItems items;
	const uint32_t* cell_scan;
	uint32_t shift, nd;
	const uint32_t* flags;
};

template <int WORDS, int NDMAX = 256>
__global__ void __launch_bounds__(MsdCfg<WORDS>::kThreads + 32, MsdCfg<WORDS>::kMinBlocks) msd_partition_kernel(const MsdPartArgs p)
{
	using S = MsdSmem<WORDS, NDMAX>;
	using R = Rec<WORDS>;
	constexpr int THREADS = S::kThreads, KPT = S::kKpt, STAGES = S::kStages;
	constexpr int DPT = NDMAX / 256;
	extern __shared__ __align__(128) uint8_t smem[];
	uint32_t* hist = reinterpret_cast<uint32_t*>(smem + S::oHist);
	uint32_t* tile_excl = reinterpret_cast<uint32_t*>(smem + S::oExcl);
	uint32_t* goff = reinterpret_cast<uint32_t*>(smem + S::oGoff);
	uint32_t* s_base = reinterpret_cast<uint32_t*>(smem + S::oBase);
	uint32_t* warp_tot = reinterpret_cast<uint32_t*>(smem + S::oWarpTot);
	uint32_t* s_geom = reinterpret_cast<uint32_t*>(smem + S::oGeom);
	uint64_t* full = reinterpret_cast<uint64_t*>(smem + S::oMbar);
	uint64_t* empty = full + STAGES;

	if (*p.flags & kMsdFlagStop) return;
	const uint32_t tid = threadIdx.x;
	const R* __restrict__ gin = reinterpret_cast<const R*>(p.in);
	R* __restrict__ gout = reinterpret_cast<R*>(p.out);
	const uint32_t n_items = *p.items.n_items;
	const uint32_t mask = p.nd - 1;

	if (tid == 0) {
#pragma unroll
		for (int i = 0; i < STAGES; ++i) { mbar_init(&full[i], 1); mbar_init(&empty[i], 1); }
		fence_mbar_init();
	}
	for (uint32_t d = tid; d < (uint32_t)NDMAX; d += blockDim.x) hist[d] = 0;
	__syncthreads();

	const uint32_t item_begin = blockIdx.x, item_end = n_items, item_step = gridDim.x;
	if (tid >= (uint32_t)THREADS) {
		const uint32_t lane = tid & 31u;
		uint32_t it = 0;
		for (uint32_t item = item_begin; item < item_end; item += item_step, ++it) {
			const uint32_t st = it % STAGES;
			if (it >= (uint32_t)STAGES) mbar_wait(&empty[st], ((it / STAGES) - 1u) & 1u);
			const MsdItemGeom g = msd_item_geom<WORDS>(p.items, item, p.nd);
#pragma unroll 8
			for (int i = 0; i < NDMAX / 32; ++i) {
				const uint32_t d = i * 32 + lane;
				s_base[st * NDMAX + d] = d < p.nd ? __ldg(p.cell_scan + g.cell0 + (uint64_t)d * g.cell_stride) : 0u;
			}
			if (lane == 0) { s_geom[st * 4 + 0] = (uint32_t)(g.lo - g.lo_al); s_geom[st * 4 + 1] = (uint32_t)(g.hi - g.lo); }
			__syncwarp();
			if (lane == 0) {
				const uint32_t bytes = g.n_load * S::kRecBytes;
				fence_proxy_async();
				mbar_arrive_expect_tx(&full[st], bytes);
				bulk_g2s(smem + S::oBuf + st * S::kBufStride, gin + g.lo_al, bytes, &full[st]);
			}
		}
		return;
	}

	const uint32_t lane = tid & 31u, warp = tid >> 5;
	uint32_t it = 0;
	for (uint32_t item = item_begin; item < item_end; item += item_step, ++it) {
		const uint32_t st = it % STAGES;
		mbar_wait(&full[st], (it / STAGES) & 1u);
		const uint32_t head = s_geom[st * 4 + 0], valid = s_geom[st * 4 + 1];
		R* buf = reinterpret_cast<R*>(smem + S::oBuf + st * S::kBufStride);

		R key[KPT];
		uint16_t rank[KPT];
#pragma unroll
		for (int r = 0; r < KPT; ++r) {
			const uint32_t j = r * THREADS + tid;
			if (j < valid) {
				key[r] = buf[head + j];
				rank[r] = (uint16_t)atomicAdd(&hist[rec_bits<WORDS>(key[r], p.shift, mask)], 1u);
			}
		}
		bar_sync_named(1, THREADS);

		uint32_t cnt[DPT], tot = 0, inc = 0;
		if (tid < 256) {
#pragma unroll
			for (int i = 0; i < DPT; ++i) { cnt[i] = hist[tid * DPT + i]; hist[tid * DPT + i] = 0; tot += cnt[i]; }
			inc = tot;
#pragma unroll
			for (int o = 1; o < 32; o <<= 1) {
				const uint32_t t = __shfl_up_sync(0xffffffffu, inc, o);
				if (lane >= (uint32_t)o) inc += t;
			}
			if (lane == 31) warp_tot[warp] = inc;
		}
		bar_sync_named(1, THREADS);
		if (tid < 256) {
			uint32_t texcl = inc - tot;
#pragma unroll
			for (int w = 0; w < 8; ++w) if ((uint32_t)w < warp) texcl += warp_tot[w];
#pragma unroll
			for (int i = 0; i < DPT; ++i) {
				tile_excl[tid * DPT + i] = texcl;
				goff[tid * DPT + i] = s_base[st * NDMAX + tid * DPT + i] - texcl;
				texcl += cnt[i];
			}
		}
		bar_sync_named(1, THREADS);

#pragma unroll
		for (int r = 0; r < KPT; ++r) {
			const uint32_t j = r * THREADS + tid;
			if (j < valid) buf[tile_excl[rec_bits<WORDS>(key[r], p.shift, mask)] + rank[r]] = key[r];
		}
		bar_sync_named(1, THREADS);

#pragma unroll
		for (int i = 0; i < KPT; ++i) {
			const uint32_t q = i * THREADS + tid;
			if (q < valid) {
				const R k = buf[q];
				gout[goff[rec_bits<WORDS>(k, p.shift, mask)] + q] = k;
			}
		}
		fence_proxy_async();
		bar_sync_named(1, THREADS);
		if (tid == 0) mbar_arrive(&empty[st]);
	}
}

struct MsdCountArgs {
	const void* in;
	MsdItems items;
	uint32_t shift, nd;
	uint16_t* cells;
	const uint32_t* flags;
};

template <int WORDS, int NDMAX = 256>
__global__ void __launch_bounds__(512) msd_count_kernel(const MsdCountArgs p)
{
	using R = Rec<WORDS>;
	__shared__ uint32_t sh[2][NDMAX];
	if (*p.flags & kMsdFlagStop) return;
	const R* __restrict__ g = reinterpret_cast<const R*>(p.in);
	const uint32_t n_items = *p.items.n_items;
	const uint32_t mask = p.nd - 1;
	const uint32_t tid = threadIdx.x;
	constexpr int U = (msd_tile<WORDS>() + 511) / 512;
	for (uint32_t d = tid; d < (uint32_t)NDMAX; d += 512) { sh[0][d] = 0; sh[1][d] = 0; }
	uint32_t item = blockIdx.x;
	MsdItemGeom gm{};
	uint32_t m = 0;
	R k[U];
	if (item < n_items) {
		gm = msd_item_geom<WORDS>(p.items, item, p.nd);
		m = (uint32_t)(gm.hi - gm.lo);
#pragma unroll
		for (int u = 0; u < U; ++u) { const uint32_t j = u * 512 + tid; if (j < m) k[u] = g[gm.lo + j]; }
	}
	__syncthreads();
	int cur = 0;
	while (item < n_items) {
#pragma unroll
		for (int u = 0; u < U; ++u) { const uint32_t j = u * 512 + tid; if (j < m) atomicAdd(&sh[cur][rec_bits<WORDS>(k[u], p.shift, mask)], 1u); }
		const MsdItemGeom done = gm;
		item += gridDim.x;
		if (item < n_items) {
			gm = msd_item_geom<WORDS>(p.items, item, p.nd);
			m = (uint32_t)(gm.hi - gm.lo);
#pragma unroll
			for (int u = 0; u < U; ++u) { const uint32_t j = u * 512 + tid; if (j < m) k[u] = g[gm.lo + j]; }
		}
		__syncthreads();
		for (uint32_t d = tid; d < (uint32_t)NDMAX; d += 512) {
			if (d < p.nd) p.cells[done.cell0 + (uint64_t)d * done.cell_stride] = (uint16_t)sh[cur][d];
			sh[cur][d] = 0;
		}
		cur ^= 1;
	}
}

constexpr int kCellChunk = 4096;

__device__ __forceinline__ void cell_load16(const uint16_t* cells, uint64_t c, uint64_t n_cells, uint32_t (&v)[16])
{
	uint4 a = make_uint4(0, 0, 0, 0), b = a;
	if (c < n_cells) { a = __ldg(reinterpret_cast<const uint4*>(cells + c)); b = __ldg(reinterpret_cast<const uint4*>(cells + c) + 1); }
	const uint32_t w[8] = {a.x, a.y, a.z, a.w, b.x, b.y, b.z, b.w};
#pragma unroll
	for (int i = 0; i < 8; ++i) {
		v[2 * i] = c + 2 * i < n_cells ? (w[i] & 0xFFFFu) : 0u;
		v[2 * i + 1] = c + 2 * i + 1 < n_cells ? (w[i] >> 16) : 0u;
	}
}

__global__ void __launch_bounds__(256) cell_reduce_kernel(const uint16_t* cells, const uint32_t* n_items, uint32_t nd, uint32_t* block_sums, const uint32_t* flags)
{
	__shared__ uint32_t s_w[8];
	if (*flags & kMsdFlagStop) return;
	const uint64_t n_cells = (uint64_t)nd * *n_items;
	const uint64_t c0 = (uint64_t)blockIdx.x * kCellChunk;
	if (c0 >= n_cells) return;
	uint32_t v[16];
	cell_load16(cells, c0 + (uint64_t)threadIdx.x * 16, n_cells, v);
	uint32_t sum = 0;
#pragma unroll
	for (int i = 0; i < 16; ++i) sum += v[i];
#pragma unroll
	for (int o = 16; o > 0; o >>= 1) sum += __shfl_down_sync(0xffffffffu, sum, o);
	if ((threadIdx.x & 31) == 0) s_w[threadIdx.x >> 5] = sum;
	__syncthreads();
	if (threadIdx.x == 0) {
		uint32_t t = 0;
		for (int w = 0; w < 8; ++w) t += s_w[w];
		block_sums[blockIdx.x] = t;
	}
}

__global__ void __launch_bounds__(1024) cell_scan_sums_kernel(uint32_t* block_sums, const uint32_t* n_items, uint32_t nd, const uint32_t* flags)
{
	__shared__ uint32_t s_w[32];
	__shared__ uint32_t carry;
	if (*flags & kMsdFlagStop) return;
	const uint64_t n_cells = (uint64_t)nd * *n_items;
	const uint32_t nb = (uint32_t)((n_cells + kCellChunk - 1) / kCellChunk);
	const uint32_t tid = threadIdx.x, lane = tid & 31, warp = tid >> 5;
	if (tid == 0) carry = 0;
	__syncthreads();
	for (uint32_t b0 = 0; b0 < nb; b0 += 1024) {
		const uint32_t b = b0 + tid;
		const uint32_t v = b < nb ? block_sums[b] : 0;
		uint32_t inc = v;
#pragma unroll
		for (int o = 1; o < 32; o <<= 1) {
			const uint32_t t = __shfl_up_sync(0xffffffffu, inc, o);
			if (lane >= (uint32_t)o) inc += t;
		}
		if (lane == 31) s_w[warp] = inc;
		__syncthreads();
		uint32_t base = carry;
		for (uint32_t w = 0; w < warp; ++w) base += s_w[w];
		if (b < nb) block_sums[b] = base + inc - v;
		__syncthreads();
		if (tid == 1023) carry = base + inc;
		__syncthreads();
	}
}

__global__ void __launch_bounds__(256) cell_scan_kernel(const uint16_t* cells, const uint32_t* n_items, uint32_t nd, const uint32_t* block_sums, uint32_t* out, const uint32_t* flags)
{
	static_assert(kCellChunk == 256 * 16, "16 consecutive cells per thread");
	__shared__ uint32_t s_w[8];
	__shared__ uint32_t s_t[kCellChunk + kCellChunk / 16];
	if (*flags & kMsdFlagStop) return;
	const uint64_t n_cells = (uint64_t)nd * *n_items;
	const uint64_t c0 = (uint64_t)blockIdx.x * kCellChunk;
	if (c0 >= n_cells) return;
	const uint32_t tid = threadIdx.x, lane = tid & 31, warp = tid >> 5;
	uint32_t v[16];
	cell_load16(cells, c0 + (uint64_t)tid * 16, n_cells, v);
	uint32_t sum = 0;
#pragma unroll
	for (int i = 0; i < 16; ++i) sum += v[i];
	uint32_t inc = sum;
#pragma unroll
	for (int o = 1; o < 32; o <<= 1) {
		const uint32_t t = __shfl_up_sync(0xffffffffu, inc, o);
		if (lane >= (uint32_t)o) inc += t;
	}
	if (lane == 31) s_w[warp] = inc;
	__syncthreads();
	uint32_t base = block_sums[blockIdx.x] + inc - sum;
	for (uint32_t w = 0; w < warp; ++w) base += s_w[w];
#pragma unroll
	for (int i = 0; i < 16; ++i) {
		s_t[tid * 17 + i] = base;
		base += v[i];
	}
	__syncthreads();
#pragma unroll
	for (int i = 0; i < 16; ++i) {
		const uint32_t j = i * 256 + tid;
		if (c0 + j < n_cells) out[c0 + j] = s_t[j + (j >> 4)];
	}
}

struct MsdBoundsArgs {
	const uint32_t* cell_scan;
	MsdItems items;
	uint32_t S, nd;
	uint64_t n;
	uint64_t* start;
	uint32_t cap;
	uint32_t* flags;
	uint32_t tile;
	uint32_t* item_base;
	uint32_t* item_seg;
	uint32_t* n_items;
};

__global__ void __launch_bounds__(256) msd_bounds_flat_kernel(const MsdBoundsArgs a)
{
	if (*a.flags & kMsdFlagStop) return;
	const uint32_t M = a.S * a.nd;
	const uint32_t m = blockIdx.x * blockDim.x + threadIdx.x;
	if (m > M) return;
	auto bound = [&](uint32_t q) -> uint64_t {
		if (q >= M) return a.n;
		const uint32_t seg = q / a.nd, d = q % a.nd;
		if (a.items.item_lo) return a.cell_scan[(uint64_t)d * *a.items.n_items];
		const uint32_t first = a.items.item_base[seg], nis = a.items.item_base[seg + 1] - first;
		return nis ? (uint64_t)a.cell_scan[(uint64_t)a.nd * first + (uint64_t)d * nis] : a.items.seg_start[seg];
	};
	const uint64_t v = bound(m);
	a.start[m] = v;
	if (a.cap && m < M && bound(m + 1) - v > a.cap) atomicOr(a.flags, kMsdFlagFallback);
}

__global__ void __launch_bounds__(1024) msd_bounds_kernel(const MsdBoundsArgs a)
{
	__shared__ uint32_t s_i[32];
	__shared__ uint32_t carry_i;
	const uint32_t tid = threadIdx.x, lane = tid & 31, warp = tid >> 5;
	if (*a.flags & kMsdFlagStop) return;
	const uint32_t M = a.S * a.nd;
	for (uint32_t m = tid; m <= M; m += 1024) {
		uint64_t v = a.n;
		if (m < M) {
			const uint32_t seg = m / a.nd, d = m % a.nd;
			if (a.items.item_lo) v = a.cell_scan[(uint64_t)d * *a.items.n_items];
			else {
				const uint32_t first = a.items.item_base[seg], nis = a.items.item_base[seg + 1] - first;
				v = nis ? (uint64_t)a.cell_scan[(uint64_t)a.nd * first + (uint64_t)d * nis] : a.items.seg_start[seg];
			}
		}
		a.start[m] = v;
	}
	__threadfence();
	__syncthreads();
	if (tid == 0) carry_i = 0;
	__syncthreads();
	bool over = false;
	for (uint32_t base = 0; base < M; base += 1024) {
		const uint32_t m = base + tid;
		uint64_t sb = 0, c = 0;
		if (m < M) { sb = a.start[m]; c = a.start[m + 1] - sb; }
		if (a.cap && c > a.cap) over = true;
		uint32_t ni = 0;
		if (a.tile && c) ni = (uint32_t)((sb + c - 1) / a.tile - sb / a.tile) + 1;
		uint32_t ii = ni;
#pragma unroll
		for (int o = 1; o < 32; o <<= 1) {
			const uint32_t t = __shfl_up_sync(0xffffffffu, ii, o);
			if (lane >= (uint32_t)o) ii += t;
		}
		if (lane == 31) s_i[warp] = ii;
		__syncthreads();
		uint32_t bi = carry_i;
		for (uint32_t w = 0; w < warp; ++w) bi += s_i[w];
		const uint32_t ei = bi + ii - ni;
		if (a.tile && m < M) a.item_base[m] = ei;
		__syncthreads();
		if (tid == 1023) carry_i = ei + ni;
		__syncthreads();
	}
	if (tid == 0 && a.tile) { a.item_base[M] = carry_i; *a.n_items = carry_i; }
	if (over) atomicOr(a.flags, kMsdFlagFallback);
	if (a.tile) {
		__syncthreads();
		for (uint32_t m = warp; m < M; m += 32) {
			const uint32_t e0 = a.item_base[m], e1 = a.item_base[m + 1];
			for (uint32_t i = e0 + lane; i < e1; i += 32) a.item_seg[i] = m;
		}
	}
}

struct MsdLocalArgs {
	const void* in;
	void* out;
	const uint64_t* start;
	uint32_t n_buckets;
	uint32_t low_bits;
	uint32_t* bucket_counter;
	const uint32_t* flags;
};

__device__ __forceinline__ uint32_t match_digit8(uint32_t d)
{
	uint32_t peers = 0xffffffffu;
#pragma unroll
	for (int b = 0; b < 8; ++b) {
		const uint32_t m = __ballot_sync(0xffffffffu, (d >> b) & 1u);
		peers &= ((d >> b) & 1u) ? m : ~m;
	}
	return peers;
}

template <int WORDS> struct MsdLocalCfg;
template <> struct MsdLocalCfg<1> { static constexpr int kThreads = 256, kKpt = 16; };
template <> struct MsdLocalCfg<2> { static constexpr int kThreads = 256, kKpt = 8; };
template <> struct MsdLocalCfg<3> { static constexpr int kThreads = 256, kKpt = 5; };
template <> struct MsdLocalCfg<4> { static constexpr int kThreads = 256, kKpt = 4; };
template <int WORDS> __host__ __device__ constexpr int msd_local_cap() { return MsdLocalCfg<WORDS>::kThreads * MsdLocalCfg<WORDS>::kKpt; }

template <int WORDS>
__global__ void __launch_bounds__(MsdLocalCfg<WORDS>::kThreads) msd_local_sort_kernel(const MsdLocalArgs p)
{
	using R = Rec<WORDS>;
	constexpr int THREADS = MsdLocalCfg<WORDS>::kThreads, KPT = MsdLocalCfg<WORDS>::kKpt, WARPS = THREADS / 32, CAP = THREADS * KPT;
	extern __shared__ __align__(16) uint8_t dsm[];
	R* buf = reinterpret_cast<R*>(dsm);
	uint32_t* whist = reinterpret_cast<uint32_t*>(dsm + (size_t)CAP * sizeof(R));
	__shared__ uint32_t tile_excl[256];
	__shared__ uint64_t warp_tot[8];
	__shared__ uint32_t s_bucket;

	if (*p.flags & kMsdFlagStop) return;
	const uint32_t tid = threadIdx.x, lane = tid & 31u, warp = tid >> 5;
	const R* __restrict__ gin = reinterpret_cast<const R*>(p.in);
	R* __restrict__ gout = reinterpret_cast<R*>(p.out);
	uint32_t* wh = whist + warp * 256;

	while (true) {
		__syncthreads();
		if (tid == 0) s_bucket = atomicAdd(p.bucket_counter, 1u);
		__syncthreads();
		const uint32_t b = s_bucket;
		if (b >= p.n_buckets) break;
		const uint64_t lo = p.start[b];
		const uint32_t m = (uint32_t)(p.start[b + 1] - lo);
		if (m == 0) continue;
		const uint32_t kpt = (m + THREADS - 1) / THREADS;
		R key[KPT];
#pragma unroll
		for (int r = 0; r < KPT; ++r) {
			if ((uint32_t)r >= kpt) break;
			const uint32_t idx = warp * (32 * kpt) + r * 32 + lane;
			if (idx < m) key[r] = gin[lo + idx];
			else {
#pragma unroll
				for (int j = 0; j < WORDS; ++j) key[r].w[j] = ~0ull;
			}
		}
		if (m > 1) {
			for (uint32_t shift = 0; shift < p.low_bits; shift += 8) {
				const uint32_t mask = (p.low_bits - shift) >= 8 ? 0xFFu : ((1u << (p.low_bits - shift)) - 1u);
#pragma unroll
				for (int i = tid; i < WARPS * 256; i += THREADS) whist[i] = 0;
				__syncthreads();
				uint32_t dg[KPT];
#pragma unroll
				for (int r = 0; r < KPT; ++r) {
					if ((uint32_t)r >= kpt) break;
					const uint32_t idx = warp * (32 * kpt) + r * 32 + lane;
					dg[r] = idx < m ? rec_bits<WORDS>(key[r], shift, mask) : mask;
					atomicAdd(&wh[dg[r]], 1u);
				}
				__syncthreads();
				uint32_t cnt = 0;
#pragma unroll
				for (int w = 0; w < WARPS; ++w) {
					const uint32_t t = whist[w * 256 + tid];
					whist[w * 256 + tid] = cnt;
					cnt += t;
				}
				const uint64_t texcl = block_excl_scan_256(cnt, warp_tot, nullptr);
				tile_excl[tid] = (uint32_t)texcl;
				__syncthreads();
				uint32_t peers[KPT];
#pragma unroll
				for (int r = 0; r < KPT; ++r) { if ((uint32_t)r >= kpt) break; peers[r] = match_digit8(dg[r]); }
#pragma unroll
				for (int r = 0; r < KPT; ++r) {
					if ((uint32_t)r >= kpt) break;
					const uint32_t d = dg[r];
					const uint32_t mm = peers[r];
					const uint32_t below = __popc(mm & lanemask_lt());
					const int leader = __ffs(mm) - 1;
					uint32_t old = 0;
					if ((int)lane == leader) {
						old = wh[d];
						wh[d] = old + __popc(mm);
					}
					old = __shfl_sync(0xffffffffu, old, leader);
					buf[tile_excl[d] + old + below] = key[r];
					__syncwarp();
				}
				__syncthreads();
#pragma unroll
				for (int r = 0; r < KPT; ++r) { if ((uint32_t)r >= kpt) break; key[r] = buf[warp * (32 * kpt) + r * 32 + lane]; }
			}
		}
#pragma unroll
		for (int r = 0; r < KPT; ++r) {
			if ((uint32_t)r >= kpt) break;
			const uint32_t idx = warp * (32 * kpt) + r * 32 + lane;
			if (idx < m) gout[lo + idx] = key[r];
		}
	}
}

}
```

Baseline: 27.04 billion.

## Compute level-1 digit totals during pack walk and scatter via atomic cursors

Level-1 top-digit histograms are now built during the pack walk and indexing kernels, using shared-memory atomics per record. The old per-tile cell histogram expand pass and its cell scan are replaced by a single bounds scan over the 256 totals. The partition expand then claims output ranges through global atomic cursors instead of a precomputed per-tile scan, and checks for overruns. This drops an expand-cells launch and a large scan, at the cost of extra per-k-mer atomics in the walk and nondeterministic placement within buckets. The heavy-leaf candidate is now chosen by majority vote over 32 samples instead of taking the first element.

```diff
diff --git a/kmc_b200/csrc/expand.cuh b/kmc_b200/csrc/expand.cuh
--- a/kmc_b200/csrc/expand.cuh
+++ b/kmc_b200/csrc/expand.cuh
@@ -42,7 +42,9 @@
 	uint64_t* item_lo1;
 	uint16_t* item_cnt1;
 	uint32_t top_shift;
-	const uint32_t* cell_scan;
+	uint32_t* l1_total;
+	uint32_t* l1_cursor;
+	const uint64_t* l1_start;
 	uint32_t mode;
 	uint32_t fshift, fprefix, fmask;
 	uint64_t* hist12;
@@ -51,7 +53,7 @@
 	const uint64_t* region_start;
 	uint32_t n_blocks;
 };
-enum : uint32_t { kExpandAll = 0, kExpandCount12 = 1, kExpandFilter = 2, kExpandScatter = 3, kExpandCells = 4, kExpandPartition = 5 };
+enum : uint32_t { kExpandAll = 0, kExpandCount12 = 1, kExpandFilter = 2, kExpandScatter = 3, kExpandPartition = 4 };
 template <int WORDS> __host__ __device__ constexpr bool expand_partition_supported() { return WORDS == 1; }
 constexpr uint32_t kExpandMaxBlocks = 512;
 constexpr uint64_t kExpandUnknownRecs = ~0ull;
@@ -60,6 +62,28 @@
 constexpr uint32_t kExpandAbortFlag = 2;
 
 __device__ __forceinline__ uint64_t tile_first_base(uint64_t pack_start, uint32_t p, uint32_t tile) { return pack_start * 4 / tile + p; }
+
+__device__ __forceinline__ void count_l1_digits(const uint8_t* sym, uint32_t x, uint32_t k, bool both_strands, uint32_t* hist)
+{
+	for (uint32_t s = 0; s <= x; s += 4) {
+		const uint32_t fw = ((uint32_t)sym[s >> 2] << 8) | sym[(s >> 2) + 1];
+		uint32_t rw = 0;
+		if (both_strands) {
+			const uint32_t b = s + k - 4, q = b >> 2;
+			const uint32_t v = (((uint32_t)sym[q] << 16) | ((uint32_t)sym[q + 1] << 8) | sym[q + 2]) >> (8u - 2u * (b & 3u));
+			const uint32_t y = __brev(v) >> 16;
+			rw = ~(((y >> 1) & 0x5555u) | ((y & 0x5555u) << 1));
+		}
+		const uint32_t n = min(x + 1 - s, 4u);
+#pragma unroll
+		for (uint32_t j = 0; j < 4; ++j) {
+			if (j < n) {
+				const uint32_t f = (fw >> (8u - 2u * j)) & 0xFFu;
+				atomicAdd(&hist[both_strands ? min(f, (rw >> (2u * j)) & 0xFFu) : f], 1u);
+			}
+		}
+	}
+}
 
 constexpr int kWalkSegBytes = 256;
 constexpr int kWalkSegs = 256;
@@ -74,10 +98,13 @@
 	extern __shared__ __align__(16) uint8_t wsm[];
 	__shared__ uint32_t s_entry[kWalkSegs], s_exit[kWalkSegs], s_w[16];
 	__shared__ uint32_t s_bad;
+	__shared__ uint32_t s_hist[256];
+	static_assert(kWalkSegs == 256, "one histogram entry per thread");
 	const uint32_t p = blockIdx.x, tid = threadIdx.x, lane = tid & 31, warp = tid >> 5;
 	const uint64_t pstart = a.pack_start[p];
 	const uint32_t len = (uint32_t)min(a.pack_start[p + 1] - pstart, (uint64_t)kWalkChunk + 1);
 	if (len > (uint32_t)kWalkChunk || len == 0) { if (tid == 0) pack_done[p] = len == 0 ? 1u : 0u; if (len == 0 && tid == 0) { a.pack_nsk[p] = 0; a.pack_nk[p] = 0; } return; }
+	s_hist[tid] = 0;
 	{
 		const uintptr_t g0 = reinterpret_cast<uintptr_t>(a.bin + pstart);
 		const uintptr_t g0a = g0 & ~(uintptr_t)15;
@@ -145,11 +172,16 @@
 			a.sk_kpre[slot + j] = kk;
 			const uint32_t tb = (kk + a.tile - 1) / a.tile;
 			if (tb * a.tile < kk + x + 1) a.tile_first[tfb + tb] = j;
+			if (a.l1_total) count_l1_digits(pk + pos + 1, x, a.k, a.both_strands != 0, s_hist);
 			kk += x + 1;
 			pos += 1 + ((x + k3) >> 2);
 			++j;
 		}
 		if (tid == 0) { a.pack_nsk[p] = tr; a.pack_nk[p] = tk; pack_done[p] = 1; }
+		if (a.l1_total) {
+			__syncthreads();
+			if (s_hist[tid]) atomicAdd(&a.l1_total[tid], s_hist[tid]);
+		}
 	}
 }
 
@@ -179,7 +211,8 @@
 	uint4 cur = walk_load_window(bin_aligned, wbase, limit, lane);
 	uint4 nxt = walk_load_window(bin_aligned, wbase + 512, limit, lane);
 	uint32_t j = 0, nk = 0, next_tile = 0;
-	uint32_t my_off = 0, my_kpre = 0;
+	uint32_t my_off = 0, my_kpre = 0, my_x = 0;
+	auto count = [&]() { if (a.l1_total) count_l1_digits(a.bin + my_off + 1, my_x, a.k, a.both_strands != 0, a.l1_total); };
 	while (pos < end) {
 		uint64_t rel = pos + shift - wbase;
 		if (rel >= 512) {
@@ -193,10 +226,11 @@
 		uint32_t w = comp == 0 ? cur.x : comp == 1 ? cur.y : comp == 2 ? cur.z : cur.w;
 		w = __shfl_sync(0xffffffffu, w, r >> 4);
 		const uint32_t x = (w >> ((r & 3u) * 8u)) & 0xFFu;
-		if (lane == (j & 31u)) { my_off = (uint32_t)pos; my_kpre = nk; }
+		if (lane == (j & 31u)) { my_off = (uint32_t)pos; my_kpre = nk; my_x = x; }
 		if ((j & 31u) == 31u) {
 			a.sk_off[slot + j - 31 + lane] = my_off;
 			a.sk_kpre[slot + j - 31 + lane] = my_kpre;
+			count();
 		}
 		if (nk + x + 1 > next_tile * a.tile) {
 			if (lane == 0) a.tile_first[tfb + next_tile] = j;
@@ -209,6 +243,7 @@
 	if (lane < (j & 31u)) {
 		a.sk_off[slot + (j & ~31u) + lane] = my_off;
 		a.sk_kpre[slot + (j & ~31u) + lane] = my_kpre;
+		count();
 	}
 	if (lane == 0) {
 		if (pos != end) atomicOr(a.status, kErrPackWalk);
@@ -222,6 +257,7 @@
 	__shared__ uint32_t s_b[32], s_k[32];
 	__shared__ uint32_t carry_b, carry_k;
 	__shared__ uint32_t s_bad;
+	__shared__ uint32_t s_hist[256];
 	const uint32_t p = blockIdx.x, tid = threadIdx.x, lane = tid & 31, warp = tid >> 5;
 	const uint64_t pstart = a.pack_start[p];
 	const uint32_t len = (uint32_t)min(a.pack_start[p + 1] - pstart, (uint64_t)0xffffffffu);
@@ -229,6 +265,7 @@
 	const uint32_t nrec = (uint32_t)min(pack_rec_start[p + 1] - r0, (uint64_t)0xffffffffu);
 	const uint64_t slot = pstart / a.min_rec_bytes;
 	const uint64_t tfb = tile_first_base(pstart, p, a.tile);
+	if (tid < 256) s_hist[tid] = 0;
 	if (tid == 0) { carry_b = 0; carry_k = 0; s_bad = 0; }
 	__syncthreads();
 	const bool too_many = (uint64_t)nrec * a.min_rec_bytes > (uint64_t)len;
@@ -254,18 +291,20 @@
 				a.sk_kpre[slot + j] = kk;
 				const uint32_t tb = (kk + a.tile - 1) / a.tile;
 				if (tb * a.tile < kk + x + 1) a.tile_first[tfb + tb] = j;
+				if (a.l1_total) count_l1_digits(a.bin + pstart + off + 1, x, a.k, a.both_strands != 0, s_hist);
 			}
 		}
 		__syncthreads();
 		if (tid == 1023) { carry_b = bb + ib; carry_k = bk + ik; }
 		__syncthreads();
 	}
+	const bool bad = too_many || s_bad || carry_b != len;
 	if (tid == 0) {
-		const bool bad = too_many || s_bad || carry_b != len;
 		if (bad) atomicOr(a.status, kErrPackWalk);
 		a.pack_nsk[p] = bad ? 0u : nrec;
 		a.pack_nk[p] = bad ? 0u : carry_k;
 	}
+	if (a.l1_total && !bad && tid < 256 && s_hist[tid]) atomicAdd(&a.l1_total[tid], s_hist[tid]);
 }
 
 __global__ void __launch_bounds__(1024) scan_packs_kernel(const ExpandArgs a)
@@ -476,14 +515,12 @@
 		if (a.flags[1] & kExpandAbortFlag) return;
 	if (tid < 256) htop[tid] = 0;
 	const uint32_t total_tiles = a.status[1];
+	auto tiles = [&]() { return MODE == kExpandPartition ? __ldg(a.status + 1) : total_tiles; };
 	Rec<WORDS>* __restrict__ out = reinterpret_cast<Rec<WORDS>*>(a.recs);
 
-	for (uint32_t g = blockIdx.x; g < total_tiles; g += gridDim.x) {
-		uint32_t digit_base = 0;
-		if constexpr (MODE == kExpandPartition)
-			if (tid < 256) digit_base = __ldg(a.cell_scan + g + (size_t)tid * total_tiles);
+	for (uint32_t g = blockIdx.x; g < tiles(); g += gridDim.x) {
 		const uint4 da = __ldg(a.tile_desc + 2 * (size_t)g), db = __ldg(a.tile_desc + 2 * (size_t)g + 1);
-		if (g + gridDim.x < total_tiles) asm volatile("prefetch.global.L2 [%0];" ::"l"(a.tile_desc + 2 * (size_t)(g + gridDim.x)));
+		if (g + gridDim.x < tiles()) asm volatile("prefetch.global.L2 [%0];" ::"l"(a.tile_desc + 2 * (size_t)(g + gridDim.x)));
 		const uint64_t slot0 = da.x;
 		const uint32_t nsk = da.y;
 		const uint32_t j_lo = da.z;
@@ -548,28 +585,14 @@
 			return extract_kmer<WORDS>(a.bin + off[j] + 1, s, a.k, a.both_strands != 0,
 				[](uintptr_t wa) { return __ldg(reinterpret_cast<const unsigned long long*>(wa)); });
 		};
-		auto top_digit_of = [&](uint32_t slot) -> uint32_t {
-			if (WORDS > 1 || !staged || a.top_shift + 8u != 2u * a.k) return rec_top_digit<WORDS>(kmer_of(slot), a.top_shift);
-			const uint32_t rel = hpre[slot >> 5] + __popc(hbits[slot >> 5] & le_mask);
-			const uint32_t B = s_bit[rel] + 2u * slot;
-			const uint32_t* sw = reinterpret_cast<const uint32_t*>(s_bytes);
-			auto byte_at = [&](uint32_t b) { const uint32_t wi = b >> 5; return __funnelshift_l(sw[wi + 1], sw[wi], b & 31u) >> 24; };
-			const uint32_t f = byte_at(B);
-			if (!a.both_strands) return f;
-			uint32_t r = ~byte_at(B + 2u * a.k - 8u) & 0xFFu;
-			r = ((r & 0x03u) << 6) | ((r & 0x0Cu) << 2) | ((r & 0x30u) >> 2) | ((r & 0xC0u) >> 6);
-			return min(f, r);
-		};
-		if constexpr (MODE == kExpandAll || MODE == kExpandCells) {
+		if constexpr (MODE == kExpandAll) {
 #pragma unroll kExpandUnroll
 			for (int i = 0; i < IPT; ++i) {
 				const uint32_t slot = i * kExpandThreads + tid;
 				if (slot < cnt) {
-					if constexpr (MODE == kExpandAll) {
-						const Rec<WORDS> r = kmer_of(slot);
-						out[obase + slot] = r;
-						atomicAdd(&htop[rec_top_digit<WORDS>(r, a.top_shift)], 1u);
-					} else atomicAdd(&htop[top_digit_of(slot)], 1u);
+					const Rec<WORDS> r = kmer_of(slot);
+					out[obase + slot] = r;
+					atomicAdd(&htop[rec_top_digit<WORDS>(r, a.top_shift)], 1u);
 				}
 			}
 			__syncthreads();
@@ -591,10 +614,11 @@
 				}
 			}
 			__syncthreads();
-			uint32_t c = 0, inc = 0;
+			uint32_t c = 0, inc = 0, base = 0;
 			if (tid < 256) {
 				c = htop[tid];
 				htop[tid] = 0;
+				if (c) base = atomicAdd(&a.l1_cursor[tid], c);
 				inc = c;
 #pragma unroll
 				for (int o = 1; o < 32; o <<= 1) {
@@ -604,14 +628,17 @@
 				if (lane == 31) warp_max[warp] = inc;
 			}
 			__syncthreads();
+			bool overrun = false;
 			if (tid < 256) {
 				uint32_t ex = inc - c;
 #pragma unroll
 				for (int w = 0; w < 8; ++w) if ((uint32_t)w < warp) ex += warp_max[w];
 				s_excl[tid] = ex;
-				s_goff[tid] = digit_base - ex;
-			}
-			__syncthreads();
+				s_goff[tid] = base - ex;
+				overrun = c && (uint64_t)base + c > (uint32_t)__ldg(a.l1_start + tid + 1);
+				if (overrun) { atomicOr(a.status, kErrRecCount); atomicOr(&a.flags[0], kExpandAbortFlag); atomicOr(&a.flags[1], kExpandAbortFlag); }
+			}
+			if (__syncthreads_or(overrun)) continue;
 			Rec<WORDS>* buf = reinterpret_cast<Rec<WORDS>*>(s_bytes);
 #pragma unroll
 			for (int i = 0; i < IPT; ++i) {
diff --git a/kmc_b200/csrc/kmc_b200.cu b/kmc_b200/csrc/kmc_b200.cu
--- a/kmc_b200/csrc/kmc_b200.cu
+++ b/kmc_b200/csrc/kmc_b200.cu
@@ -38,7 +38,7 @@
 
 thread_local std::string g_create_error;
 
-enum { kHistNone = 0, kHistTiles = 1, kHistCells = 2 };
+enum { kHistNone = 0, kHistTiles = 1, kHistTotals = 2 };
 
 struct ZeroBlock {
 	uint64_t hist[kHistRows][256];
@@ -50,6 +50,8 @@
 	uint32_t heavy_count[2];
 	uint32_t heavy_list[kHeavyListCap];
 	uint32_t leaf_group_sum[kMaxLeaves / 1024];
+	uint32_t l1_total[256];
+	uint32_t l1_cursor[256];
 };
 
 static_assert(sizeof(ZeroBlock) % 4 == 0, "zeroed word by word");
@@ -249,11 +251,9 @@
 	const uint32_t grid = std::min<uint32_t>(max_tiles, (uint32_t)(ctx->sm_count * (a.mode == kExpandPartition ? std::max(ctx->occ_expand_part, 1) : ctx->occ_expand)));
 	switch (a.mode) {
 	case kExpandAll: expand_kernel<WORDS, kExpandAll><<<grid, ExpandCfg<WORDS>::kThreads, 0, st>>>(a); break;
-	case kExpandCells:
 	case kExpandPartition:
 		if constexpr (expand_partition_supported<WORDS>()) {
-			if (a.mode == kExpandCells) expand_kernel<WORDS, kExpandCells><<<grid, ExpandCfg<WORDS>::kThreads, 0, st>>>(a);
-			else expand_kernel<WORDS, kExpandPartition><<<grid, ExpandCfg<WORDS>::kThreads, 0, st>>>(a);
+			expand_kernel<WORDS, kExpandPartition><<<grid, ExpandCfg<WORDS>::kThreads, 0, st>>>(a);
 			break;
 		} else return fail(ctx, KMCB200_ERR_INVALID, "no level-1 partition expansion for %d-word records", WORDS);
 	case kExpandCount12: expand_kernel<WORDS, kExpandCount12><<<grid, ExpandCfg<WORDS>::kThreads, 0, st>>>(a); break;
@@ -353,12 +353,12 @@
 	if (n_tiles64 > 0x7fffffffull || n >= (1ull << 32)) return fail(ctx, KMCB200_ERR_INVALID, "bin too large: %llu records", (unsigned long long)n);
 	const uint32_t n_tiles = (uint32_t)n_tiles64;
 	const bool msd = msd_path(ctx, n, key_bits);
-	if (hist_mode == kHistCells && !msd) return fail(ctx, KMCB200_ERR_INVALID, "the records of this bin were not expanded");
+	if (hist_mode == kHistTotals && !msd) return fail(ctx, KMCB200_ERR_INVALID, "the records of this bin were not expanded");
 	const uint32_t top_shift = key_bits - 8;
 	if (int rc = ensure(ctx, s.desc, s.desc_cap, (size_t)n_tiles * 256, true)) return rc;
 	if (msd) if (int rc = ensure_msd<WORDS>(ctx, s, n, n_packs, choose_nd2<WORDS>(ctx, n, plan != nullptr))) return rc;
 
-	const bool hist_ready = hist_mode == kHistTiles || hist_mode == kHistCells;
+	const bool hist_ready = hist_mode == kHistTiles || hist_mode == kHistTotals;
 	if (hist_mode == kHistNone) if (int rc = zero_async(ctx, s.zero, sizeof(ZeroBlock), st)) return rc;
 	int iv = 0;
 	CU(cudaEventRecord(s.ev_pass[0], st));
@@ -379,9 +379,9 @@
 		const int local_smem = msd_local_cap<WORDS>() * 8 * WORDS + (MsdLocalCfg<WORDS>::kThreads / 32) * 1024;
 
 		MsdItems items1{};
-		if (hist_ready) {
+		if (hist_mode == kHistTiles) {
 			items1.item_lo = s.msd_item_lo1; items1.item_cnt = s.msd_item_cnt1; items1.n_items = &s.zero->status[1];
-		} else {
+		} else if (hist_mode == kHistNone) {
 			msd_setup_kernel<<<1, 1, 0, st>>>(s.msd_seg1, s.msd_item_base1, &s.zero->msd_n_items[0], n, MTILE);
 			items1.seg_start = s.msd_seg1; items1.item_base = s.msd_item_base1; items1.item_seg = s.msd_item_seg2 ;
 			items1.n_items = &s.zero->msd_n_items[0];
@@ -390,28 +390,34 @@
 			msd_count_kernel<WORDS><<<(uint32_t)std::min<size_t>(max_items1, (size_t)ctx->sm_count * 4), 512, 0, st>>>(c1);
 			ctx->launches += 2;
 		}
-		if (int rc = launch_cell_scan(ctx, s, items1.n_items, 256, max_items1, never, st)) return rc;
-		s.pass_names[iv] = "msd_scan_L1"; CU(cudaEventRecord(s.ev_pass[++iv], st));
+		if (hist_mode != kHistTotals) {
+			if (int rc = launch_cell_scan(ctx, s, items1.n_items, 256, max_items1, never, st)) return rc;
+			s.pass_names[iv] = "msd_scan_L1"; CU(cudaEventRecord(s.ev_pass[++iv], st));
+		}
 		MsdBoundsArgs b1{};
 		b1.cell_scan = s.msd_cell_scan; b1.items = items1; b1.S = 1; b1.nd = 256; b1.n = n; b1.start = s.msd_start2;
 		b1.cap = b2 == 0 ? cap : 0; b1.flags = flags;
 		b1.tile = b2 > 0 ? MTILE : 0; b1.item_base = s.msd_item_base2; b1.item_seg = s.msd_item_seg2; b1.n_items = &s.zero->msd_n_items[1];
-		MsdPartArgs p1{};
-		p1.in = a; p1.out = b; p1.items = items1; p1.cell_scan = s.msd_cell_scan; p1.shift = top_shift; p1.nd = 256;
-		p1.flags = never;
-		if (hist_mode == kHistCells) {
+		if (hist_mode == kHistTotals) {
+			b1.l1_total = s.zero->l1_total; b1.l1_cursor = s.zero->l1_cursor; b1.status = s.zero->status;
+			msd_bounds_kernel<<<1, 1024, 0, st>>>(b1);
+			ctx->launches++;
 			ExpandArgs ea = s.expand_args;
-			ea.mode = kExpandPartition; ea.recs = b; ea.cell_scan = s.msd_cell_scan;
+			ea.mode = kExpandPartition; ea.recs = b; ea.l1_cursor = s.zero->l1_cursor; ea.l1_start = s.msd_start2;
 			if (int rc = launch_expand<WORDS>(ctx, ea, st)) return rc;
 			s.pass_names[iv] = "expand_scatter_L1";
+			CU(cudaEventRecord(s.ev_pass[++iv], st));
 		} else {
+			MsdPartArgs p1{};
+			p1.in = a; p1.out = b; p1.items = items1; p1.cell_scan = s.msd_cell_scan; p1.shift = top_shift; p1.nd = 256;
+			p1.flags = never;
 			msd_partition_kernel<WORDS><<<pgrid1, MsdCfg<WORDS>::kThreads + 32, MsdSmem<WORDS>::kBytes, st>>>(p1);
 			ctx->launches++;
 			s.pass_names[iv] = "msd_partition_L1";
-		}
-		CU(cudaEventRecord(s.ev_pass[++iv], st));
-		msd_bounds_kernel<<<1, 1024, 0, st>>>(b1);
-		ctx->launches++;
+			CU(cudaEventRecord(s.ev_pass[++iv], st));
+			msd_bounds_kernel<<<1, 1024, 0, st>>>(b1);
+			ctx->launches++;
+		}
 		if (b2 > 0) {
 			MsdItems items2{};
 			items2.seg_start = s.msd_start2; items2.item_base = s.msd_item_base2; items2.item_seg = s.msd_item_seg2; items2.n_items = &s.zero->msd_n_items[1];
@@ -559,8 +565,9 @@
 	bool big_pack = !(n_packs && pack_bytes) && size > (uint64_t)kWalkChunk;
 	if (n_packs && pack_bytes) for (uint32_t i = 0; i < n_packs && !big_pack; ++i) big_pack = pack_bytes[i] > (uint64_t)kWalkChunk;
 	s.last_n_packs = np;
-	const bool cells = em.mode == kExpandAll || em.mode == kExpandCells;
-	s.hist_mode = em.mode == kExpandAll ? kHistTiles : em.mode == kExpandCells ? kHistCells : kHistNone;
+	const uint32_t mode = em.mode;
+	const bool msd_items = mode == kExpandAll || mode == kExpandPartition;
+	s.hist_mode = mode == kExpandAll ? kHistTiles : mode == kExpandPartition ? kHistTotals : kHistNone;
 
 	if (int rc = ensure(ctx, s.sk_off, s.sk_off_cap, size / min_rec + 2)) return rc;
 	if (int rc = ensure(ctx, s.sk_kpre, s.sk_kpre_cap, size / min_rec + 2)) return rc;
@@ -578,19 +585,20 @@
 	a.tile_desc = s.tile_desc;
 	a.status = s.zero->status; a.flags = s.zero->msd_flags;
 	a.recs = d_recs;
-	a.mode = em.mode; a.fshift = em.fshift; a.fprefix = em.fprefix; a.fmask = em.fmask; a.hist12 = em.hist12; a.out_counter = em.out_counter;
+	a.mode = mode; a.fshift = em.fshift; a.fprefix = em.fprefix; a.fmask = em.fmask; a.hist12 = em.hist12; a.out_counter = em.out_counter;
 	a.blk_of_prefix = em.blk_of_prefix; a.region_start = em.region_start; a.n_blocks = em.n_blocks;
-	if (cells) {
+	if (msd_items)
 		if (int rc = DISPATCH_WORDS(ctx, ensure_msd, ctx, s, n_rec, np, DISPATCH_WORDS(ctx, choose_nd2, ctx, n_rec, ctx->use_leaf))) return rc;
-		a.cells1 = s.msd_cells; a.item_lo1 = s.msd_item_lo1; a.item_cnt1 = s.msd_item_cnt1;
-	} else { a.cells1 = nullptr; a.item_lo1 = nullptr; a.item_cnt1 = nullptr; }
+	if (mode == kExpandAll) { a.cells1 = s.msd_cells; a.item_lo1 = s.msd_item_lo1; a.item_cnt1 = s.msd_item_cnt1; }
+	else { a.cells1 = nullptr; a.item_lo1 = nullptr; a.item_cnt1 = nullptr; }
 	a.top_shift = std::max(2u * k, 8u) - 8u;
-	a.cell_scan = nullptr;
-	if (em.mode == kExpandCells) s.expand_args = a;
+	a.l1_total = mode == kExpandPartition ? s.zero->l1_total : nullptr;
+	a.l1_cursor = nullptr; a.l1_start = nullptr;
+	if (mode == kExpandPartition) s.expand_args = a;
 
 	bin_init_kernel<<<64, 256, 0, st>>>(reinterpret_cast<uint32_t*>(s.zero), (uint32_t)(sizeof(ZeroBlock) / 4), reinterpret_cast<uint32_t*>(zero_lut),
 		(size_t)ctx->lut_entries * 2, reinterpret_cast<uint32_t*>(zero_result));
-	if (s.have_extras && cells) {
+	if (s.have_extras && msd_items) {
 		index_from_extras_kernel<<<np, 1024, 0, st>>>(a, s.d_extras, s.d_pack_rec);
 		ctx->launches += 2;
 		big_pack = false;
@@ -610,6 +618,7 @@
 		CU(cudaEventRecord(s.ev_walk, st));
 		CU(cudaStreamWaitEvent(st_expand, s.ev_walk, 0));
 	}
+	if (mode == kExpandPartition) return 0;
 	return DISPATCH_WORDS(ctx, launch_expand, ctx, a, st_expand);
 }
 
@@ -798,7 +807,7 @@
 	if (int rc = ensure(ctx, s.recs_a, s.recs_a_cap, n_rec * rec_bytes)) return rc;
 	if (int rc = ensure(ctx, s.recs_b, s.recs_b_cap, n_rec * rec_bytes)) return rc;
 	ExpandMode em;
-	if (expand_partition_supported<1>() && ctx->words == 1 && n_rec < (1ull << 32) && msd_path(ctx, n_rec, 2u * ctx->prm.kmer_len)) em.mode = kExpandCells;
+	if (expand_partition_supported<1>() && ctx->words == 1 && n_rec < (1ull << 32) && msd_path(ctx, n_rec, 2u * ctx->prm.kmer_len)) em.mode = kExpandPartition;
 	if (int rc = stage_expand(ctx, s, d_bin, size, n_rec, pack_bytes, n_packs, s.recs_a, st, em, packs_uploaded, d_lut, d_result, st_walk)) return rc;
 	CU(cudaEventRecord(s.ev_expand, st));
 	s.ran_expand = true;
diff --git a/kmc_b200/csrc/leaf_warp.cuh b/kmc_b200/csrc/leaf_warp.cuh
--- a/kmc_b200/csrc/leaf_warp.cuh
+++ b/kmc_b200/csrc/leaf_warp.cuh
@@ -198,7 +198,15 @@
 		uint32_t n_eq = 0, m_rest = m;
 		const unsigned long long* __restrict__ g = reinterpret_cast<const unsigned long long*>(recs) + lo;
 		if (m > kLwHeavy && m <= kLwMaxHeavyLeaf) {
-			cand = __ldg(g);
+			{
+				const uint64_t smp = __ldg(g + (uint64_t)lane * m / 32);
+				uint32_t votes = 0;
+				for (int i = 0; i < 32; ++i) votes += __shfl_sync(FULL, smp, i) == smp;
+				uint32_t best = (votes << 5) | (31u - lane);
+#pragma unroll
+				for (int o = 16; o > 0; o >>= 1) best = max(best, __shfl_xor_sync(FULL, best, o));
+				cand = __shfl_sync(FULL, smp, 31u - (best & 31u));
+			}
 			for (uint32_t j0 = 0; j0 < m; j0 += 128) {
 				uint64_t v[4];
 #pragma unroll
diff --git a/kmc_b200/csrc/msd_sort.cuh b/kmc_b200/csrc/msd_sort.cuh
--- a/kmc_b200/csrc/msd_sort.cuh
+++ b/kmc_b200/csrc/msd_sort.cuh
@@ -1,5 +1,6 @@
 #pragma once
 #include "common.cuh"
+#include "expand.cuh"
 #include "radix_sort.cuh"
 
 namespace kmcb {
@@ -400,6 +401,9 @@
 	uint32_t* item_base;
 	uint32_t* item_seg;
 	uint32_t* n_items;
+	const uint32_t* l1_total;
+	uint32_t* l1_cursor;
+	uint32_t* status;
 };
 
 __global__ void __launch_bounds__(256) msd_bounds_flat_kernel(const MsdBoundsArgs a)
@@ -427,6 +431,27 @@
 	const uint32_t tid = threadIdx.x, lane = tid & 31, warp = tid >> 5;
 	if (*a.flags & kMsdFlagStop) return;
 	const uint32_t M = a.S * a.nd;
+	if (a.l1_total) {
+		const uint32_t c = tid < M ? a.l1_total[tid] : 0u;
+		uint32_t inc = c;
+#pragma unroll
+		for (int o = 1; o < 32; o <<= 1) {
+			const uint32_t t = __shfl_up_sync(0xffffffffu, inc, o);
+			if (lane >= (uint32_t)o) inc += t;
+		}
+		if (lane == 31) s_i[warp] = inc;
+		__syncthreads();
+		uint32_t ex = inc - c;
+		for (uint32_t w = 0; w < warp; ++w) ex += s_i[w];
+		if (tid < M) { a.start[tid] = ex; a.l1_cursor[tid] = ex; }
+		if (tid == M) a.start[M] = a.n;
+		if (tid == M - 1) carry_i = ex + c;
+		__syncthreads();
+		if (carry_i != a.n) {
+			if (tid == 0) { atomicOr(a.status, kErrRecCount); atomicOr(&a.flags[0], kMsdFlagAbort); atomicOr(&a.flags[1], kMsdFlagAbort); }
+			return;
+		}
+	} else
 	for (uint32_t m = tid; m <= M; m += 1024) {
 		uint64_t v = a.n;
 		if (m < M) {
```

Result: faster. 30.84 billion, median of 6 (+14.1%).
